# jianzhnie/RLZero

Measured on AMD Instinct MI355X. Metric: mcts_sims_per_sec, higher is better.
Workload: dtype f32 net (hi + lo f16 operand pairs on the f16 MFMA pipe, f32 accumulation) / f64 tree

## Files before the change

profiles/microbench/delta_resident_phases.py:

```python
import ctypes, os, sys
sys.path.insert(0, os.environ.get('GRAFT_REPO_ROOT', '.'))
import rlzero_amd._hip as H
H.library_path = lambda: os.environ.get('RZ_NETPROF_LIB') or os.path.join(os.path.dirname(os.path.abspath(__file__)), 'librlzero_netprof.so')
import rlzero_amd._build as B
B.needs_build = lambda: False
import numpy as np, torch
from rlzero_amd.engine import HipNetEvaluator, MCTSEngine
from rlzero_amd.games.gomoku.policy_value_net import PolicyValueNet
lib = H.load()
NAMES = [(0, 'leaf + changed cells'), (1, 'distances, requests, ranks'), (3, 'maps, base records'), (4, 'bar'), (5, 'conv1'), (6, 'bar'), (7, 'conv2'),
         (9, 'bar + conv3 + heads'), (10, 'bar'), (11, 'features'), (12, 'bar'), (16, 'value layer'), (17, 'expand + backup'),
         (2, 'sel: root record'), (8, 'sel: root scan / answer'), (13, 'sel: level-0 cell'), (14, 'sel: deeper levels'), (15, 'sel: terminal test + leaf stores'),
         (18, 'selection (rest: hand-over)'), (19, 'wave 1: pre-scan'), (20, 'wave 1: wait behind it')]
VALUES = '--values' in sys.argv[1:]
if VALUES:
    import rlzero_amd.route as _R
    _R.policy_on_demand = lambda *a, **k: True
sizes = [int(a) for a in sys.argv[1:] if a != '--values'] or [1, 256, 512]
for games in sizes:
    torch.manual_seed(0)
    net = PolicyValueNet(15).to('cuda:0')
    ev = HipNetEvaluator(net, 15, 'cuda:0', max_boards=games)
    sims = 800
    eng = MCTSEngine(15, 5, n_games=games, n_playout=sims, device='cuda:0', add_noise=True)
    eng.reset_games()
    assert ev.resident_ok(eng) and ev.resident_delta_ok(eng)
    rng = np.random.default_rng(0)
    for ply in range(6):
        eng.sim_chunk(ev, 40)
        visits = eng.root_visits()
        moves = np.array([int(rng.choice(np.flatnonzero(v > 0))) for v in visits], dtype=np.int32)
        eng.advance(moves)
        eng.step(moves)
    a, b = torch.cuda.Event(enable_timing=True), torch.cuda.Event(enable_timing=True)
    ev.hip.delta_stats(reset=True)
    a.record(); eng.sim_chunk(ev, sims); b.record(); torch.cuda.synchronize()
    assert (eng.search_launches[True] > 0) == VALUES and (eng.search_launches[False] > 0) != VALUES
    st = ev.hip.delta_stats()
    out = (ctypes.c_longlong * 24)()
    assert lib.rz_net_debug_profile(out) == 0
    us = 1e3 * a.elapsed_time(b) / sims
    total = out[23] / sims
    print('%d games, %d simulations: %.2f us per simulation of a game (events, bases included), %d cycles (%.2f GHz); %.2f conv3 / %.2f conv2 tiles, %.2f changed cells per leaf, %d leaves without a base' % (
        games, sims, us, total, total / us / 1e3, st['tiles3'] / max(1, st['delta'] + st['no_base']), st['tiles2'] / max(1, st['delta'] + st['no_base']),
        st['cells'] / max(1, st['delta'] + st['no_base']), st['no_base']))
    print('   ' + '  '.join('%s=%d' % (nm, out[k] / sims) for k, nm in NAMES) + '  prescans=%d' % st['prescans'], flush=True)
    eng.close(); ev.hip.close()
```

rlzero_amd/csrc/rz_delta.h:

```cpp

#pragma once

#include <hip/hip_runtime.h>

#include <stdint.h>

#include "rlzero_hip.h"
#include "rz_gather.h"
#include "rz_net_dev.h"
#include "rz_net_rows.h"
#include "rz_net_split.h"
#include "rz_trace.h"
#include "rz_tree.h"
#include "rz_window.h"

#ifndef RZ_DELTA_TREE_PRIO
#define RZ_DELTA_TREE_PRIO 1
#endif
#ifndef RZ_DELTA_PRO_PRIO
#define RZ_DELTA_PRO_PRIO 0
#endif
#ifndef RZ_DELTA_PRESCAN
#define RZ_DELTA_PRESCAN 1
#endif

namespace {

namespace dl {

using sp::f16x4;
using sp::f16x8;
typedef const __attribute__((address_space(3))) f16x8 *lds_frag;
typedef const __attribute__((address_space(3))) uint32_t *lds_u32;
typedef __attribute__((address_space(3))) f16x4 *lds_h4;
typedef __attribute__((address_space(3))) f32x4 *lds_v4;

constexpr int kC1Slots = 128, kC2Slots = 164;
constexpr int kT1 = 4, kT2 = 8, kT3 = 8;
constexpr int kMaxD = 4;
constexpr int P1 = rt::Geo<32>::pos_bytes, P2 = rt::Geo<64>::pos_bytes;
constexpr int kGrid = kRowW * kRowW;
constexpr int kShareFloats = kT3 * 4 * 96;
constexpr int kHeadW = 128 * 6 * 4 + 128 * 4 + 32;
constexpr int kOffC1 = sp::kInPieceBytes, kOffC2 = kOffC1 + kC1Slots * P1, kOffZero = kOffC2 + kC2Slots * P2, kOffHead = kOffZero + P2,
              kOffMap1 = kOffHead + kHeadW, kOffMap2 = kOffMap1 + kGrid * 4, kOffList = kOffMap2 + kGrid * 4,
              kLdsBytes = kOffList + 3 * 128 * 2;
static_assert(kShareFloats * 4 <= kC1Slots * P1, "the shares lie inside conv1's records (dead behind conv2)");
constexpr int kWinSets = rzw::kRadii * rzw::kWords, kWinLds = kWinSets * 8 + kWinSets * 4 + 16;
static_assert(2 * (kLdsBytes + 512 * 4 + 4 * 64 * 4 + 80 + kWinLds + (int)sizeof(rzt::RootPre) + 512) <= 160 * 1024,
              "two workgroups per CU, also of the resident search (value row, K-quarter sums, leaf, window sets, root pre-scan)");
static_assert(kOffC1 % 16 == 0 && kOffZero % 16 == 0 && kOffHead % 16 == 0 && kOffMap1 % 16 == 0, "alignment");

constexpr int kCells = RZ_MAX_BOARD_SIZE * RZ_MAX_BOARD_SIZE;
struct BaseHdr {
    uint64_t stones[2 * RZ_BOARD_WORDS];
    int32_t to_move, valid, pad[2];
};
constexpr size_t kBaseC2 = (size_t)kCells * 128, kBaseV = kBaseC2 + (size_t)kCells * 256, kBaseBytes = kBaseV + (size_t)6 * kCells * 4;

struct DeltaArgs {
    BaseHdr *hdr;
    char *recs;
    const uint8_t *active;
    float *feat32;
    unsigned *stats;
    int mode;
    int bw_rcp;
    const uint64_t *win;
};

__device__ __forceinline__ uint32_t lds_addr(const void *p) {
    return (uint32_t)(uintptr_t)((const __attribute__((address_space(3))) char *)p);
}

constexpr int unit_tiles(int nt) { return nt <= 3 ? nt : (nt + 1) / 2; }
constexpr int units_of(int nt) { return (nt + unit_tiles(nt) - 1) / unit_tiles(nt); }

template <int CIN, int NT, int UT>
__device__ __forceinline__ void read_unit(f16x8 (&b)[UT][2], const uint32_t (&rec)[NT][3], int h, int dy, int c) {
#pragma unroll
    for (int i = 0; i < UT; ++i) {
        const int t = h * UT + i;
        if (t < NT) {
            const uint32_t r = rec[t][dy] + (uint32_t)(c * 64);
            b[i][0] = *(lds_frag)(uintptr_t)r;
            b[i][1] = *(lds_frag)(uintptr_t)(r + CIN * 2);
        }
    }
}
template <int TM, int NT, int UT>
__device__ __forceinline__ void mfma_unit(f32x4 (&acc)[TM][NT], const f16x8 (&a)[TM][2], const f16x8 (&b)[UT][2], int h) {
#pragma unroll
    for (int combo = 0; combo < 3; ++combo)
#pragma unroll
        for (int i = 0; i < UT; ++i) {
            const int t = h * UT + i;
            if (t < NT) {
#pragma unroll
                for (int m = 0; m < TM; ++m)
                    acc[m][t] = __builtin_amdgcn_mfma_f32_16x16x32_f16(a[m][combo == 2], b[i][combo == 1], acc[m][t], 0, 0, 0);
            }
        }
}
template <int NT>
__device__ __forceinline__ void lookup(uint32_t (&rec)[NT][3], lds_u32 map, const int (&pos19)[NT], int dx, int g) {
#pragma unroll
    for (int t = 0; t < NT; ++t)
#pragma unroll
        for (int dy = 0; dy < 3; ++dy) rec[t][dy] = map[pos19[t] + dx + dy * kRowW] + (uint32_t)(g * 16);
}

template <int NT>
__device__ __forceinline__ void conv2_g(lds_u32 map, const int (&pos19)[NT], int lane, const f16x8 (&a2)[9][1][2], f32x4 (&acc)[1][NT]) {
    static_assert(NT <= 4, "one unit per step");
    const int g = lane >> 4;
#pragma unroll
    for (int t = 0; t < NT; ++t) acc[0][t] = f32x4{0.f, 0.f, 0.f, 0.f};
    constexpr int AHEAD = NT <= 2 ? 2 : 1;
    uint32_t rec[3][NT][3];
    f16x8 b[AHEAD + 1][NT][2];
#pragma unroll
    for (int dx = 0; dx < 3; ++dx) lookup<NT>(rec[dx], map, pos19, dx, g);
#pragma unroll
    for (int u = 0; u < AHEAD; ++u) read_unit<32, NT, NT>(b[u], rec[u / 3], 0, u % 3, 0);
#pragma unroll
    for (int u = 0; u < 9; ++u) {
        const int dx = u / 3, dy = u % 3;
        if (u + AHEAD < 9) read_unit<32, NT, NT>(b[(u + AHEAD) % (AHEAD + 1)], rec[(u + AHEAD) / 3], 0, (u + AHEAD) % 3, 0);
        mfma_unit<1, NT, NT>(acc, a2[dy * 3 + dx], b[u % (AHEAD + 1)], 0);
        __builtin_amdgcn_sched_barrier(0);
    }
}

#ifndef RZ_DELTA_RING6_UPTO
#define RZ_DELTA_RING6_UPTO 2
#endif
constexpr int ring3(int nt) { return nt <= RZ_DELTA_RING6_UPTO ? 6 : 3; }
__device__ __forceinline__ void load_a3(f16x8 (&a)[2][2], __amdgpu_buffer_rsrc_t w_rsrc, int lane, int dx, int j) {
    using G = rt::Geo<64>;
    const int c = j / 3, dy = j % 3;
#pragma unroll
    for (int m = 0; m < 2; ++m)
#pragma unroll
        for (int p = 0; p < 2; ++p)
            a[m][p] = sp::load_w(w_rsrc, lane * 16, dx * (G::chunks * 2048) + ((m * G::steps + dy * 3 * G::chunks + c) * 2 + p) * 1024);
}
template <int NT>
__device__ __forceinline__ void conv3_g(lds_u32 map, const uint16_t *list3, const void *wts, int lane, bool sync, f32x4 (&acc)[2][NT]) {
    static_assert(NT <= 6, "two units per step");
    constexpr int R = ring3(NT), H = units_of(NT);
    const int n = lane & 15, g = lane >> 4;
    const __amdgpu_buffer_rsrc_t w_rsrc = __builtin_amdgcn_make_buffer_rsrc(const_cast<void *>(wts), 0, 0x7fffffff, 0x00020000);
    f16x8 a3[R][2][2];
#pragma unroll
    for (int j = 0; j < R - 1; ++j) load_a3(a3[j], w_rsrc, lane, 0, j);
    if (sync) __syncthreads();
    int pos19[NT];
#pragma unroll
    for (int t = 0; t < NT; ++t) pos19[t] = (int)list3[16 * t + n] - 19;
#pragma unroll
    for (int m = 0; m < 2; ++m)
#pragma unroll
        for (int t = 0; t < NT; ++t) acc[m][t] = f32x4{0.f, 0.f, 0.f, 0.f};
    uint32_t rec[NT][3], recn[NT][3];
#ifndef RZ_DELTA_AHEAD3_SMALL
#define RZ_DELTA_AHEAD3_SMALL 1
#endif
    constexpr int UT = unit_tiles(NT), AH = UT <= 2 ? RZ_DELTA_AHEAD3_SMALL : 1, NB = AH + 1;
    static_assert((6 * H) % NB == 0 && AH <= H * 6, "a unit's registers are a constant of the unrolled body");
    f16x8 b[NB][UT][2];
    lookup<NT>(rec, map, pos19, 0, g);
#pragma unroll
    for (int u = 0; u < AH; ++u) read_unit<64, NT, UT>(b[u], rec, u % H, (u / H) % 3, u / H / 3);
#pragma unroll 1
    for (int dx = 0; dx < 3; ++dx) {
        lookup<NT>(recn, map, pos19, dx < 2 ? dx + 1 : 2, g);
#pragma unroll
        for (int u = 0; u < 6 * H; ++u) {
            const int j = u / H, h = u % H;
            if (h == 0) {
                const int jj = j + R - 1, dx2 = jj < 6 ? dx : (dx < 2 ? dx + 1 : 2);
                load_a3(a3[jj % R], w_rsrc, lane, dx2, jj % 6);
            }
            {
                const int v = u + AH;
                if (v < 6 * H) read_unit<64, NT, UT>(b[v % NB], rec, v % H, (v / H) % 3, v / H / 3);
                else read_unit<64, NT, UT>(b[v % NB], recn, (v - 6 * H) % H, ((v - 6 * H) / H) % 3, (v - 6 * H) / H / 3);
            }
            mfma_unit<2, NT, UT>(acc, a3[j % R], b[u % NB], h);
            __builtin_amdgcn_sched_barrier(0);
        }
#pragma unroll
        for (int t = 0; t < NT; ++t)
#pragma unroll
            for (int dy = 0; dy < 3; ++dy) rec[t][dy] = recn[t][dy];
    }
}

template <int T, int O = 6>
__device__ __forceinline__ void reduce_scatter(const float (&vals)[O * T], float (&out)[O * T / 4]) {
    float r1[O * T / 2];
#pragma unroll
    for (int i = 0; i < O * T / 2; ++i) {
        const auto sw = __builtin_amdgcn_permlane16_swap(__float_as_uint(vals[i]), __float_as_uint(vals[O * T / 2 + i]), false, false);
        r1[i] = __uint_as_float(sw[0]) + __uint_as_float(sw[1]);
    }
#pragma unroll
    for (int i = 0; i < O * T / 4; ++i) {
        const auto sw = __builtin_amdgcn_permlane32_swap(__float_as_uint(r1[i]), __float_as_uint(r1[O * T / 4 + i]), false, false);
        out[i] = __uint_as_float(sw[0]) + __uint_as_float(sw[1]);
    }
}

template <int NT>
__device__ __forceinline__ void conv2_tiles(lds_u32 map1, lds_u32 map2, const uint16_t *list2, int n2, int lane, int wave, const f16x8 (&a2)[9][1][2],
                                            f32x4 bias2, float k2) {
    const int n = lane & 15, g = lane >> 4;
    int pos19[NT];
#pragma unroll
    for (int t = 0; t < NT; ++t) pos19[t] = (int)list2[16 * t + n] - 19;
    f32x4 acc[1][NT];
    conv2_g<NT>(map1, pos19, lane, a2, acc);
#pragma unroll
    for (int t = 0; t < NT; ++t) {
        if (16 * t + n < n2) {
            const uint32_t rec = map2[pos19[t] + kRowW + 1] + (uint32_t)((16 * wave + 4 * g) * 2);
            float z[4];
#pragma unroll
            for (int j = 0; j < 4; ++j) z[j] = fmaxf(fmaf(acc[0][t][j], k2, bias2[j]), 0.0f);
            f16x4 hi, lo;
            sp::split4(z, hi, lo);
            *(lds_h4)(uintptr_t)rec = hi;
            *(lds_h4)(uintptr_t)(rec + 128) = lo;
        }
    }
}

template <int NT, int OLO = 0, int OHI = 6>
__device__ __forceinline__ void conv3_tiles(lds_u32 map2, const uint16_t *list3, const void *wts, int lane, int wave, bool sync,
                                            const char *headw, float k3, float *shares) {
    constexpr int T = NT <= 4 ? 4 : 8, O = OHI - OLO;
    static_assert(OLO % 2 == 0 && OHI % 2 == 0 && 0 <= OLO && OLO < OHI && OHI <= 6, "pairs of outputs");
    const int n = lane & 15, g = lane >> 4;
    float vals[O * T];
    {
        f32x4 acc[2][NT];
        conv3_g<NT>(map2, list3, wts, lane, sync, acc);
        f32x4 hwr[2][6], b3r[2];
#pragma unroll
        for (int m = 0; m < 2; ++m) {
            const int c0 = 32 * wave + 16 * m + 4 * g;
#pragma unroll
            for (int i = 0; i < 6; ++i) hwr[m][i] = *reinterpret_cast<const f32x4 *>(headw + (c0 * 6 + 4 * i) * 4);
            b3r[m] = *reinterpret_cast<const f32x4 *>(headw + 128 * 6 * 4 + c0 * 4);
        }
#pragma unroll
        for (int t = 0; t < T; ++t) {
            f32x2 v2[3] = {f32x2{0.0f, 0.0f}, f32x2{0.0f, 0.0f}, f32x2{0.0f, 0.0f}};
            if (t < NT) {
#pragma unroll
                for (int m = 0; m < 2; ++m)
#pragma unroll
                    for (int j = 0; j < 4; ++j) {
                        const float hv = fmaxf(fmaf(acc[m][t < NT ? t : 0][j], k3, b3r[m][j]), 0.0f);
#pragma unroll
                        for (int o2 = OLO / 2; o2 < OHI / 2; ++o2) {
                            const int e = 6 * j + 2 * o2;
                            v2[o2] = __builtin_elementwise_fma(f32x2{hwr[m][e >> 2][e & 3], hwr[m][e >> 2][(e & 3) + 1]}, f32x2{hv, hv}, v2[o2]);
                        }
                    }
            }
#pragma unroll
            for (int o = OLO; o < OHI; ++o) vals[t * O + o - OLO] = v2[o >> 1][o & 1];
        }
    }
    float mine[O * T / 4];
    reduce_scatter<T, O>(vals, mine);
    const int t0 = (T / 2) * (g & 1) + (T / 4) * (g >> 1);
#pragma unroll
    for (int i = 0; i < O * T / 4; ++i)
        if (t0 + i / O < NT) shares[((t0 + i / O) * 4 + wave) * 96 + (OLO + i % O) * 16 + n] = mine[i];
}

struct Leaf {
    f16x4 cell_planes;
    const char *base;
    int dys[kMaxD], dxs[kMaxD];
    _Float16 *dst16;
    float *vdst;
    float *dst32;
    const uint64_t *sets;
    uint16_t *gtab;
    bool deferred, store_head;
};
struct Layers {
    float k1, k2, k3, act1, act2, act3;
    const char *t2p, *t3p;
};
#ifdef RZ_NET_PROFILE
struct Prof { long long acc[24], t; };
#else
struct Prof {};
#endif

__device__ __forceinline__ void init_maps(char *lds, int tid) {
    uint32_t *map1 = reinterpret_cast<uint32_t *>(lds + kOffMap1);
    const uint32_t zaddr = lds_addr(lds + kOffZero);
    for (int i = tid; i < 2 * kGrid; i += 256) map1[i] = zaddr;
    if (tid < 3 * 128 / 2) reinterpret_cast<uint32_t *>(lds + kOffList)[tid] = 19u | (19u << 16);
}

__device__ __forceinline__ int cell_dist(int cy, int cx, int pass, const int (&dys)[kMaxD], const int (&dxs)[kMaxD], int BH, int BW) {
    int dist = 1000;
    if (pass < 0) {
#pragma unroll
        for (int i = 0; i < kMaxD; ++i) {
            const int ady = cy > dys[i] ? cy - dys[i] : dys[i] - cy, adx = cx > dxs[i] ? cx - dxs[i] : dxs[i] - cx;
            const int d = ady > adx ? ady : adx;
            dist = d < dist ? d : dist;
        }
    } else {
        const int y0 = 8 * (pass >> 1), x0 = 8 * (pass & 1);
        const int y1 = (y0 + 8 < BH ? y0 + 8 : BH) - 1, x1 = (x0 + 8 < BW ? x0 + 8 : BW) - 1;
        const int ddy = cy < y0 ? y0 - cy : (cy > y1 ? cy - y1 : 0), ddx = cx < x0 ? x0 - cx : (cx > x1 ? cx - x1 : 0);
        dist = ddy > ddx ? ddy : ddx;
    }
    return dist;
}

constexpr int kOutside = 1 << 30;
__device__ __forceinline__ f32x4 load_rec(__amdgpu_buffer_rsrc_t rsrc, int off) {
    return __builtin_bit_cast(f32x4, __builtin_amdgcn_raw_buffer_load_b128(rsrc, off, 0, 0));
}

__device__ __forceinline__ uint64_t uni64(uint64_t v) {
    return ((uint64_t)(unsigned)__builtin_amdgcn_readfirstlane((int)(v >> 32)) << 32) | (unsigned)__builtin_amdgcn_readfirstlane((int)v);
}

__device__ __forceinline__ int lane_below(uint64_t word) {
    return (int)__builtin_amdgcn_mbcnt_hi((unsigned)(word >> 32), __builtin_amdgcn_mbcnt_lo((unsigned)word, 0u));
}
static_assert(rzg::kC1Max == kC1Slots && rzg::kC2Max == kC2Slots && rzg::kC1Bytes * kCells == (int)kBaseC2 && rzg::kOutside == kOutside,
              "rz_gather.h's records are the base's and the budget is this file's");
static_assert(rzg::kC1Bytes <= P1 && rzg::kC2Bytes <= P2, "a record fits its LDS slot");

template <bool SETS, int OLO = 0, int OHI = 6>
__device__ __forceinline__ int delta_passes(const NetDev &nd, const DeltaArgs &da, char *lds, int tid0, int wave, const Leaf &leaf, const Layers &ly,
                                            f32x4 headv, bool &use_delta, Prof &prof) {
    char *in0 = lds, *c1 = lds + kOffC1, *c2 = lds + kOffC2, *zrec = lds + kOffZero, *headw = lds + kOffHead;
    uint32_t *map1 = reinterpret_cast<uint32_t *>(lds + kOffMap1), *map2 = reinterpret_cast<uint32_t *>(lds + kOffMap2);
    uint16_t *list1 = reinterpret_cast<uint16_t *>(lds + kOffList), *list2 = list1 + 128, *list3 = list2 + 128;
    float *shares = reinterpret_cast<float *>(c1);
    const int mode = da.mode, BH = nd.BH, BW = nd.BW, S = nd.S;
    const float k1 = ly.k1, k2 = ly.k2, k3 = ly.k3, act1 = ly.act1, act2 = ly.act2, act3 = ly.act3;
    const char *t2p = ly.t2p, *t3p = ly.t3p;
    const char *base = leaf.base;
    const f16x4 cell_planes = leaf.cell_planes;
    const int (&dys)[kMaxD] = leaf.dys, (&dxs)[kMaxD] = leaf.dxs;
    _Float16 *dst16 = leaf.dst16;
    float *vdst = leaf.vdst, *dst32 = leaf.dst32;
    const bool deferred = leaf.deferred, store_head = leaf.store_head;
    const uint32_t zaddr = lds_addr(zrec);
    int n_conv3_tiles = 0, n_conv2_tiles = 0;
#ifdef RZ_NET_PROFILE
    long long (&prof_acc)[24] = prof.acc, &prof_t = prof.t;
#endif
    for (int pass = use_delta ? -1 : 0; pass < 4; ++pass) {
        int tid = tid0;
        asm volatile("" : "+v"(tid));
        const int lane = tid & 63, g = lane >> 4;
        const int cy = (tid * da.bw_rcp) >> 16, cx = tid - cy * BW;
        const bool is_cell = tid < S;
        const int mypos = is_cell ? (cy + 1) * kRowW + cx + 1 : 0;
        if (RZ_DELTA_PRO_PRIO) __builtin_amdgcn_s_setprio(RZ_DELTA_PRO_PRIO);
        const int th[5] = {pass < 0 ? 1 : 2, pass < 0 ? 2 : 1, pass < 0 ? 3 : 0, pass < 0 ? 3 : 2, pass < 0 ? 4 : 1};
        bool f[5];
        uint64_t own[5];
        const bool handed = SETS && pass < 0;
        int rank[5], tot[5];
        if (handed) {
#pragma unroll
            for (int k = 0; k < 5; ++k) {
                own[k] = uni64(leaf.sets[4 * (th[k] - 1) + wave]);
                f[k] = (own[k] >> lane) & 1ull;
            }
            const int *cnt = reinterpret_cast<const int *>(leaf.sets + kWinSets);
#pragma unroll
            for (int k = 0; k < 5; ++k) {
                int before = 0, all = 0;
#pragma unroll
                for (int w = 0; w < 4; ++w) {
                    const int c = __builtin_amdgcn_readfirstlane(cnt[4 * (th[k] - 1) + w]);
                    all += c;
                    before += w < wave ? c : 0;
                }
                rank[k] = before + (int)__builtin_amdgcn_mbcnt_hi((unsigned)(own[k] >> 32), __builtin_amdgcn_mbcnt_lo((unsigned)own[k], 0u));
                tot[k] = all;
            }
        } else {
            const int dist = cell_dist(cy, cx, pass, dys, dxs, BH, BW);
#pragma unroll
            for (int k = 0; k < 5; ++k) f[k] = is_cell && dist <= th[k];
        }
        const bool g1 = pass < 0 && f[3] && !f[0], g2 = pass < 0 && f[4] && !f[1];
        const __amdgpu_buffer_rsrc_t b_rsrc = __builtin_amdgcn_make_buffer_rsrc(const_cast<char *>(base), 0, kBaseBytes, 0x00020000);
        f32x4 r1[8], r2[16];
        f32x4 q1[rzg::kC1Rounds], q2[rzg::kC2Rounds];
        uint32_t d1[rzg::kC1Rounds], d2[rzg::kC2Rounds];
        if constexpr (SETS) {
            uint16_t *tab = leaf.gtab;
            uint64_t ws[rzw::kRadii][rzg::kWords];
#pragma unroll
            for (int r = 0; r < rzw::kRadii; ++r)
#pragma unroll
                for (int w = 0; w < rzg::kWords; ++w) ws[r][w] = leaf.sets[4 * r + w];
            int n1 = 0, s1 = 0, n2 = 0, s2 = 0;
#pragma unroll
            for (int w = 0; w < rzg::kWords; ++w) {
                const uint64_t h1 = rzg::held(ws[2][w], ws[0][w]), h2 = rzg::held(ws[3][w], ws[1][w]);
                const int cell = 64 * w + lane;
                const int p1 = rzg::c1_place(n1 + lane_below(h1), wave), p2 = rzg::c2_place(n2 + lane_below(h2), wave);
                const uint16_t e1 = rzg::entry(cell, s1 + lane_below(ws[2][w])), e2 = rzg::entry(cell, s2 + lane_below(ws[3][w]));
                if (handed && ((h1 >> lane) & 1ull) && p1 >= 0) tab[p1] = e1;
                if (handed && ((h2 >> lane) & 1ull) && p2 >= 0) tab[p2] = e2;
                n1 += rzg::popcount(h1), s1 += rzg::popcount(ws[2][w]);
                n2 += rzg::popcount(h2), s2 += rzg::popcount(ws[3][w]);
            }
            const uint32_t c1a = lds_addr(c1), c2a = lds_addr(c2);
#pragma unroll
            for (int i = 0; i < rzg::kC1Rounds; ++i) {
                const int j = rzg::c1_record(i, wave, lane), chunk = rzg::c1_chunk(lane);
                const uint16_t e = tab[rzg::c1_index(j)];
                const bool has = handed && rzg::c1_has(j, n1);
                d1[i] = has ? c1a + (uint32_t)rzg::dst(rzg::entry_slot(e), chunk, P1) : zaddr + 16u * (uint32_t)chunk;
                q1[i] = load_rec(b_rsrc, rzg::c1_src(has, rzg::entry_cell(e), chunk));
            }
#pragma unroll
            for (int i = 0; i < rzg::kC2Rounds; ++i) {
                const int j = rzg::c2_record(i, wave, lane), chunk = rzg::c2_chunk(lane);
                const uint16_t e = tab[rzg::c2_index(j)];
                const bool has = handed && rzg::c2_has(j, n2);
                d2[i] = has ? c2a + (uint32_t)rzg::dst(rzg::entry_slot(e), chunk, P2) : zaddr + 16u * (uint32_t)chunk;
                q2[i] = load_rec(b_rsrc, rzg::c2_src(has, rzg::entry_cell(e), chunk, (int)kBaseC2));
            }
        } else {
            const int o1 = g1 ? tid * 128 : kOutside, o2 = g2 ? (int)kBaseC2 + tid * 256 : kOutside;
#pragma unroll
            for (int i = 0; i < 8; ++i) r1[i] = load_rec(b_rsrc, o1 + 16 * i);
#pragma unroll
            for (int i = 0; i < 16; ++i) r2[i] = load_rec(b_rsrc, o2 + 16 * i);
        }
        float bv[6];
        {
            const int ov = pass < 0 && is_cell && !f[2] ? (int)kBaseV + tid * 4 : kOutside;
#pragma unroll
            for (int o = OLO; o < OHI; ++o) bv[o] = __builtin_bit_cast(float, __builtin_amdgcn_raw_buffer_load_b32(b_rsrc, ov + o * kCells * 4, 0, 0));
        }
        sp::f16x8 a1[3][2];
        f32x4 bias1[4];
        if constexpr (SETS) {
            const __amdgpu_buffer_rsrc_t s_rsrc = __builtin_amdgcn_make_buffer_rsrc(const_cast<f32x4 *>(nd.s1), 0, 6 * 64 * 16, 0x00020000);
            const __amdgpu_buffer_rsrc_t o_rsrc = __builtin_amdgcn_make_buffer_rsrc(const_cast<float *>(nd.b1), 0, 32 * 4, 0x00020000);
            const bool runs = !handed || 32 * wave < tot[0];
            const int so = runs ? lane * 16 : kOutside, bo = runs ? 16 * (lane >> 5) : kOutside;
#pragma unroll
            for (int ky = 0; ky < 3; ++ky)
#pragma unroll
                for (int p_ = 0; p_ < 2; ++p_) a1[ky][p_] = sp::load_w(s_rsrc, so, (ky * 2 + p_) * 1024);
#pragma unroll
            for (int gg = 0; gg < 4; ++gg) bias1[gg] = load_rec(o_rsrc, bo + 32 * gg);
        } else if (32 * wave < 32 * kT1) {
#pragma unroll
            for (int ky = 0; ky < 3; ++ky)
#pragma unroll
                for (int p_ = 0; p_ < 2; ++p_) a1[ky][p_] = __builtin_bit_cast(sp::f16x8, nd.s1[(ky * 2 + p_) * 64 + lane]);
#pragma unroll
            for (int gg = 0; gg < 4; ++gg) bias1[gg] = *reinterpret_cast<const f32x4 *>(nd.b1 + 8 * gg + 4 * (lane >> 5));
        }
        f32x4 bias2 = *reinterpret_cast<const f32x4 *>(nd.b2 + 16 * wave + 4 * g);
        if (!handed) {
            int before[5] = {0, 0, 0, 0, 0}, all[5] = {0, 0, 0, 0, 0};
            unsigned long long own[5] = {0ull, 0ull, 0ull, 0ull, 0ull};
#pragma unroll
            for (int b = 0; b < 4; ++b) {
                const int cell = 64 * b + lane, by = (cell * da.bw_rcp) >> 16, bx = cell - by * BW;
                const int d = cell_dist(by, bx, pass, dys, dxs, BH, BW);
#pragma unroll
                for (int k = 0; k < 5; ++k) {
                    const unsigned long long m = __ballot(cell < S && d <= th[k]);
                    const int c = __popcll(m);
                    all[k] += c;
                    before[k] += b < wave ? c : 0;
                    own[k] = b == wave ? m : own[k];
                }
            }
#pragma unroll
            for (int k = 0; k < 5; ++k) {
                rank[k] = before[k] + (int)__builtin_amdgcn_mbcnt_hi((unsigned)(own[k] >> 32), __builtin_amdgcn_mbcnt_lo((unsigned)own[k], 0u));
                tot[k] = all[k];
            }
        }
        NET_TICK(1);
        if (pass < 0 && (tot[0] > 32 * kT1 || tot[1] > 16 * kT2 || tot[2] > 16 * kT3 || tot[3] > kC1Slots || tot[4] > kC2Slots)) {
            use_delta = false;
            continue;
        }
        uint32_t rec1 = 0, rec2 = 0;
        if (f[3]) {
            rec1 = lds_addr(c1 + rank[3] * P1);
            map1[mypos] = rec1;
        }
        if (f[4]) {
            rec2 = lds_addr(c2 + rank[4] * P2);
            map2[mypos] = rec2;
        }
        if (f[0]) list1[rank[0]] = (uint16_t)mypos;
        if (f[1]) list2[rank[1]] = (uint16_t)mypos;
        if (f[2]) list3[rank[2]] = (uint16_t)mypos;
        if (pass <= 0 && is_cell) *reinterpret_cast<f16x4 *>(in0 + ((cy + 1) * sp::kInCols + (cx + 1)) * 8) = cell_planes;
        if (pass <= 0 && store_head && tid < 226) reinterpret_cast<f32x4 *>(headw)[tid] = headv;
        if constexpr (SETS) {
#pragma unroll
            for (int i = 0; i < rzg::kC1Rounds; ++i) *(lds_v4)(uintptr_t)d1[i] = q1[i];
#pragma unroll
            for (int i = 0; i < rzg::kC2Rounds; ++i) *(lds_v4)(uintptr_t)d2[i] = q2[i];
        } else {
            if (g1) {
#pragma unroll
                for (int i = 0; i < 8; ++i) *(lds_v4)(uintptr_t)(rec1 + 16 * i) = r1[i];
            }
            if (g2) {
#pragma unroll
                for (int i = 0; i < 16; ++i) *(lds_v4)(uintptr_t)(rec2 + 16 * i) = r2[i];
            }
        }
        __builtin_amdgcn_sched_barrier(0);
        f16x8 a2[9][1][2];
        {
            const __amdgpu_buffer_rsrc_t w_rsrc = __builtin_amdgcn_make_buffer_rsrc(const_cast<char *>(t2p), 0, 0x7fffffff, 0x00020000);
#pragma unroll
            for (int tap = 0; tap < 9; ++tap)
#pragma unroll
                for (int p = 0; p < 2; ++p) a2[tap][0][p] = sp::load_w(w_rsrc, lane * 16, (tap * 2 + p) * 1024);
        }
        NET_TICK(3);
        __syncthreads();
        NET_TICK(4);

        if (32 * wave < tot[0]) {
            const int n32 = lane & 31, h = lane >> 5, idx = 32 * wave + n32;
            const int pos = list1[idx];
            const int py = (pos * 3641) >> 16, px = pos - py * kRowW;
            typedef const __attribute__((address_space(3))) f16x4 *lds_half;
            const lds_half q = (lds_half)(in0 + ((py - 1) * sp::kInCols + (px - 1) + 2 * h) * 8);
            sp::f16x8 b1[3];
#pragma unroll
            for (int ky = 0; ky < 3; ++ky) {
                const int o = ky * sp::kInCols;
                const f16x4 lo4 = q[o], hi4 = q[o + 1];
                b1[ky] = __builtin_shufflevector(lo4, hi4, 0, 1, 2, 3, 4, 5, 6, 7);
            }
            sp::f32x16 acc1;
#pragma unroll
            for (int r = 0; r < 16; ++r) acc1[r] = 0.0f;
#pragma unroll
            for (int ky = 0; ky < 3; ++ky)
#pragma unroll
                for (int combo = 0; combo < 3; combo += 2)
                    acc1 = __builtin_amdgcn_mfma_f32_32x32x16_f16(a1[ky][combo == 2], b1[ky], acc1, 0, 0, 0);
            if (idx < tot[0]) {
                const uint32_t rec = map1[pos] + (uint32_t)(4 * h * 2);
#pragma unroll
                for (int gg = 0; gg < 4; ++gg) {
                    float z[4];
#pragma unroll
                    for (int j = 0; j < 4; ++j) z[j] = fmaxf(fmaf(acc1[4 * gg + j], k1, bias1[gg][j] * act1), 0.0f);
                    f16x4 hi, lo;
                    sp::split4(z, hi, lo);
                    *(lds_h4)(uintptr_t)(rec + 8 * gg * 2) = hi;
                    *(lds_h4)(uintptr_t)(rec + 8 * gg * 2 + 64) = lo;
                }
            }
        }
        NET_TICK(5);
        __syncthreads();
        NET_TICK(6);
        if (mode == 1 && f[0]) {
            f32x4 *dstp = reinterpret_cast<f32x4 *>(const_cast<char *>(base) + (size_t)tid * 128);
#pragma unroll
            for (int i = 0; i < 8; ++i) dstp[i] = *(lds_v4)(uintptr_t)(rec1 + 16 * i);
        }

        if (RZ_DELTA_PRO_PRIO) __builtin_amdgcn_s_setprio(0);
        const int nt3 = (tot[2] + 15) >> 4;
        {
            const lds_u32 m1 = (lds_u32)map1, m2 = (lds_u32)map2;
            const int nt2 = (tot[1] + 15) >> 4;
            n_conv2_tiles += nt2;
            for (int t0 = 0; t0 < nt2; t0 += 4) {
                const uint16_t *l2 = list2 + 16 * t0;
                const int left = tot[1] - 16 * t0;
                switch (nt2 - t0) {
                    case 1: conv2_tiles<1>(m1, m2, l2, left, lane, wave, a2, bias2 * act2, k2); break;
                    case 2: conv2_tiles<2>(m1, m2, l2, left, lane, wave, a2, bias2 * act2, k2); break;
                    case 3: conv2_tiles<3>(m1, m2, l2, left, lane, wave, a2, bias2 * act2, k2); break;
                    default: conv2_tiles<4>(m1, m2, l2, left, lane, wave, a2, bias2 * act2, k2); break;
                }
            }
        }
        NET_TICK(7);

        {
            const lds_u32 m2 = (lds_u32)map2;
            n_conv3_tiles += nt3;
            const int first = nt3 <= 6 ? nt3 : 4;
            switch (first) {
                case 0: __syncthreads(); break;
                case 1: conv3_tiles<1, OLO, OHI>(m2, list3, t3p, lane, wave, true, headw, k3, shares); break;
                case 2: conv3_tiles<2, OLO, OHI>(m2, list3, t3p, lane, wave, true, headw, k3, shares); break;
                case 3: conv3_tiles<3, OLO, OHI>(m2, list3, t3p, lane, wave, true, headw, k3, shares); break;
                case 4: conv3_tiles<4, OLO, OHI>(m2, list3, t3p, lane, wave, true, headw, k3, shares); break;
                case 5: conv3_tiles<5, OLO, OHI>(m2, list3, t3p, lane, wave, true, headw, k3, shares); break;
                default: conv3_tiles<6, OLO, OHI>(m2, list3, t3p, lane, wave, true, headw, k3, shares); break;
            }
            if (nt3 == 7) conv3_tiles<3, OLO, OHI>(m2, list3 + 64, t3p, lane, wave, false, headw, k3, shares + 4 * 4 * 96);
            else if (nt3 >= 8) conv3_tiles<4, OLO, OHI>(m2, list3 + 64, t3p, lane, wave, false, headw, k3, shares + 4 * 4 * 96);
        }
        NET_TICK(9);
        __syncthreads();
        NET_TICK(10);
        if (mode == 1 && f[1]) {
            f32x4 *dstp = reinterpret_cast<f32x4 *>(const_cast<char *>(base) + kBaseC2 + (size_t)tid * 256);
#pragma unroll
            for (int i = 0; i < 16; ++i) dstp[i] = *(lds_v4)(uintptr_t)(rec2 + 16 * i);
        }

        if (is_cell && (pass < 0 || f[2])) {
            const float *share = shares + (rank[2] >> 4) * 4 * 96 + (rank[2] & 15);
            float *basev = mode == 1 ? reinterpret_cast<float *>(const_cast<char *>(base) + kBaseV) : nullptr;
#pragma unroll
            for (int o = OLO; o < OHI; ++o) {
                float v;
                if (f[2]) {
                    float s = share[o * 16];
#pragma unroll
                    for (int w = 1; w < 4; ++w) s += share[w * 96 + o * 16];
                    v = fmaxf(s + reinterpret_cast<const float *>(headw + 128 * 7 * 4)[o], 0.0f);
                } else {
                    v = bv[o];
                }
                if (mode == 1) {
                    basev[o * kCells + tid] = v;
                    continue;
                }
                if (dst32) dst32[o * S + tid] = v;
                if (deferred && o >= 4) {
                    vdst[(o - 4) * S + tid] = v;
                } else if (dst16) {
                    const int k = (o < 4 ? o : o - 4) * S + tid;
                    const int step = (o < 4 ? 0 : nd.groups_act) + (k >> 4);
                    const float z = v * act3;
                    const _Float16 zh = (_Float16)z;
                    _Float16 *q = dst16 + (size_t)step * 1024 + (k & 15);
                    q[0] = zh;
                    q[512] = (_Float16)(z - (float)zh);
                }
            }
        }
        if (f[3]) map1[mypos] = zaddr;
        if (f[4]) map2[mypos] = zaddr;
        NET_TICK(11);
        if (pass < 0) break;
        __syncthreads();
    }
    return n_conv3_tiles | (n_conv2_tiles << 16);
}

__device__ __forceinline__ f16x4 planes_of(const uint64_t (&ls)[8], int tid, int tm_eff, bool has_last, int lc, int par_count) {
    f16x4 cell_planes;
    const int word = (tid >> 6) & 3, bit = tid & 63;
    uint64_t w0 = 0ull, w1 = 0ull;
#pragma unroll
    for (int w = 0; w < 4; ++w) {
        const uint64_t mk = word == w ? ~0ull : 0ull;
        w0 |= ls[w] & mk;
        w1 |= ls[4 + w] & mk;
    }
    const bool s0 = (w0 >> bit) & 1ull, s1 = (w1 >> bit) & 1ull;
    const bool mine = tm_eff == 0 ? s0 : s1, theirs = tm_eff == 0 ? s1 : s0;
    const _Float16 one = (_Float16)sp::kObsScale, zero = (_Float16)0.0f;
    cell_planes[0] = mine ? one : zero;
    cell_planes[1] = theirs ? one : zero;
    cell_planes[2] = (has_last && tid == lc) ? one : zero;
    cell_planes[3] = (par_count & 1) ? zero : one;
    return cell_planes;
}

__device__ __forceinline__ bool changed_cells(const uint64_t (&ls)[8], const uint64_t (&rs)[8], int nst, int tm, int lc, bool has_last, bool base_ok, int h_tm,
                                              int bw_rcp, int BW, int (&dys)[kMaxD], int (&dxs)[kMaxD], int &parity, int &nD) {
    bool use_delta = false;
    {
        bool sup = true;
        int nroot = 0;
        uint64_t D[4] = {0ull, 0ull, 0ull, 0ull};
#pragma unroll
        for (int q = 0; q < 8; ++q) {
            sup = sup && (rs[q] & ~ls[q]) == 0ull;
            nroot += __popcll(rs[q]);
            D[q & 3] |= rs[q] ^ ls[q];
        }
#pragma unroll
        for (int w = 0; w < 4; ++w) D[w] |= (has_last && lc >= 0 && (lc >> 6) == w) ? 1ull << (lc & 63) : 0ull;
        parity = (nst - nroot) & 1;
        nD = __popcll(D[0]) + __popcll(D[1]) + __popcll(D[2]) + __popcll(D[3]);
        use_delta = base_ok && sup && tm == (h_tm ^ parity) && nD <= kMaxD;
#pragma unroll
        for (int i = 0; i < kMaxD; ++i) {
            const bool z0 = D[0] == 0ull, z1 = D[1] == 0ull, z2 = D[2] == 0ull;
            const int w = !z0 ? 0 : !z1 ? 1 : !z2 ? 2 : 3;
            const uint64_t word = !z0 ? D[0] : !z1 ? D[1] : !z2 ? D[2] : D[3];
            const bool any = word != 0ull;
            const int cell = 64 * w + __builtin_ctzll(word | (1ull << 63));
            const uint64_t rest = word & (word - 1ull);
#pragma unroll
            for (int k = 0; k < 4; ++k) D[k] = k == w ? rest : D[k];
            const int y = (cell * bw_rcp) >> 16;
            dys[i] = any ? y : -100;
            dxs[i] = any ? cell - y * BW : -100;
        }
    }
    return use_delta;
}

template <bool TRACE>
__global__ __launch_bounds__(256, 2) void k_trunk_delta(NetDev nd, LeafBits leaves, _Float16 *__restrict__ feat16, int n_boards,
                                                        DeferredOut later, DeltaArgs da) {
    __shared__ __attribute__((aligned(16))) char lds[kLdsBytes];
    const int board = blockIdx.x;
    const int mode = da.mode;
    const int game = mode == 1 ? board >> 1 : board, par_b = mode == 1 ? board & 1 : 0;
    unsigned long long trace_t0 = 0;
    if (TRACE) trace_t0 = rz_trace_now();
    Prof prof;
#ifdef RZ_NET_PROFILE
    for (int i = 0; i < 24; ++i) prof.acc[i] = 0;
    prof.t = __builtin_readcyclecounter();
    const long long prof_k0 = prof.t;
    long long (&prof_acc)[24] = prof.acc, &prof_t = prof.t;
#endif
    const int tid0 = threadIdx.x, wave = __builtin_amdgcn_readfirstlane(tid0 >> 6);
    const int BW = nd.BW, S = nd.S;
    Layers ly;
    ly.t2p = reinterpret_cast<const char *>(nd.t2) + (size_t)wave * rt::Geo<32>::steps * 2 * 1024;
    ly.t3p = reinterpret_cast<const char *>(nd.t3) + (size_t)(2 * wave) * rt::Geo<64>::steps * 2 * 1024;
    f32x4 headv = tid0 < 192 ? reinterpret_cast<const f32x4 *>(nd.whp)[tid0] : reinterpret_cast<const f32x4 *>(nd.b3)[(tid0 - 192) & 31];
    {
        const float *bh = nd.bh + (tid0 == 225 ? 4 : 0);
        const f32x4 hbv = {bh[0], bh[1], tid0 == 225 ? 0.0f : bh[2], tid0 == 225 ? 0.0f : bh[3]};
        headv = (tid0 == 224 || tid0 == 225) ? hbv : headv;
    }
    ly.k1 = nd.s_inv[2], ly.k2 = nd.s_inv[0], ly.k3 = nd.s_inv[1];
    ly.act1 = nd.s_inv[5], ly.act2 = nd.s_inv[6], ly.act3 = nd.s_inv[7];

    const uint64_t *sb = leaves.stones + (size_t)game * 8;
    const BaseHdr *hd = da.hdr + game;
    uint64_t ls[8], rs[8];
    int nst = 0;
#pragma unroll
    for (int q = 0; q < 8; ++q) {
        ls[q] = sb[q];
        rs[q] = hd->stones[q];
        nst += __popcll(ls[q]);
    }
    const int tm = leaves.to_move[game];
    const int lc_raw = (mode == 1 ? leaves.to_move : leaves.last)[game];
    const int lc = mode == 1 ? -1 : lc_raw;
    const int h_tm = hd->to_move, h_valid = hd->valid;
    const int is_active = da.active[game];
    const bool deferred = later.slot_of != nullptr;
    const int slot_ = (deferred ? later.slot_of : leaves.to_move)[deferred ? board : game];
    const int tm_eff = tm ^ par_b;
    const int par_count = nst + par_b;
    const bool has_last = mode != 1 && nst > 0;

    Leaf leaf;
    int parity = 0, nD = 0;
    bool use_delta = changed_cells(ls, rs, nst, tm, lc, has_last, mode == 0 && h_valid != 0, h_tm, da.bw_rcp, BW, leaf.dys, leaf.dxs, parity, nD);
    leaf.base = da.recs + ((size_t)game * 2 + (mode == 1 ? par_b : parity)) * kBaseBytes;
    leaf.cell_planes = planes_of(ls, tid0, tm_eff, has_last, lc, par_count);

    leaf.dst16 = nullptr;
    leaf.vdst = nullptr;
    if (mode != 1 && deferred) {
        leaf.dst16 = (feat16 != nullptr && slot_ < later.n_slots) ? feat16 + (size_t)slot_ * later.slot_halfs + (size_t)(board >> 5) * nd.groups_act * 1024 + (board & 31) * 16 : nullptr;
        leaf.vdst = later.valfeat + (size_t)board * later.vf_ld;
    }
    if (mode != 1 && !deferred && feat16 != nullptr)
        leaf.dst16 = feat16 + ((size_t)(board >> 5) * (nd.groups_act + nd.groups_val) * 1024 + (board & 31) * 16);
    leaf.dst32 = (mode != 1 && da.feat32 != nullptr) ? da.feat32 + (size_t)board * 6 * S : nullptr;
    leaf.sets = nullptr, leaf.gtab = nullptr;
    leaf.deferred = deferred;
    leaf.store_head = true;

    {
        const f32x4 zero = {0.f, 0.f, 0.f, 0.f};
        f32x4 *z = reinterpret_cast<f32x4 *>(lds);
        for (int i = tid0; i < sp::kInPieceBytes / 16; i += 256) z[i] = zero;
        if (tid0 < P2 / 16) reinterpret_cast<f32x4 *>(lds + kOffZero)[tid0] = zero;
        init_maps(lds, tid0);
    }
    if (mode == 0 && is_active == 0) return;
    __syncthreads();
    NET_TICK(0);
    const int n_tiles = delta_passes<false>(nd, da, lds, tid0, wave, leaf, ly, headv, use_delta, prof);
    const int n_conv3_tiles = n_tiles & 0xffff;

    if (mode == 1 && par_b == 0 && tid0 == 0) {
        BaseHdr *h = da.hdr + game;
#pragma unroll
        for (int q = 0; q < 8; ++q) h->stones[q] = sb[q];
        h->to_move = tm;
        h->valid = 1;
    }
    if (da.stats != nullptr && tid0 == 0 && mode != 1) {
        atomicAdd(da.stats + (use_delta ? 0 : 1), 1u);
        atomicAdd(da.stats + 2, (unsigned)n_conv3_tiles);
        atomicAdd(da.stats + 3, (unsigned)nD);
        atomicAdd(da.stats + 4, (unsigned)(n_tiles >> 16));
    }
#ifdef RZ_NET_PROFILE
    if (blockIdx.x == 0 && tid0 == 0) {
        for (int i = 0; i < 24; ++i) net_prof[i] = prof_acc[i];
        net_prof[23] = __builtin_readcyclecounter() - prof_k0;
        net_prof[22] = n_conv3_tiles;
    }
#endif
    if (TRACE && tid0 == 0) rz_trace_write(later.trace, RZ_TRACE_TRUNK, deferred ? slot_ : 0, board, trace_t0);
}

__device__ __forceinline__ void windows_store(uint64_t row, bool use_delta, int parity, int nD, int lane, uint64_t *ws) {
    unsigned lo = (unsigned)row, hi = (unsigned)(row >> 32);
    {
        const auto a = __builtin_amdgcn_permlane16_swap(lo, lo, false, false), b = __builtin_amdgcn_permlane16_swap(hi, hi, false, false);
        lo = a[0] | a[1];
        hi = b[0] | b[1];
    }
    {
        const auto a = __builtin_amdgcn_permlane32_swap(lo, lo, false, false), b = __builtin_amdgcn_permlane32_swap(hi, hi, false, false);
        lo = a[0] | a[1];
        hi = b[0] | b[1];
    }
    const uint64_t v = ((uint64_t)hi << 32) | lo;
    int *cnt = reinterpret_cast<int *>(ws + kWinSets);
    if (lane < kWinSets) {
        ws[lane] = v;
        cnt[lane] = __popcll(v);
    }
    if (lane == 0) cnt[kWinSets] = (use_delta ? 1 : 0) | (parity << 1) | (nD << 8);
}
__device__ __forceinline__ void leaf_windows(const uint64_t *leaf_lds, const uint64_t (&rs)[8], bool base_ok, int h_tm, const DeltaArgs &da, int BW,
                                             int lane, uint64_t *ws) {
    uint64_t ls[8];
    int nst = 0;
#pragma unroll
    for (int q = 0; q < 8; ++q) {
        ls[q] = uni64(leaf_lds[q]);
        nst += __popcll(ls[q]);
    }
    const int tm = __builtin_amdgcn_readfirstlane(reinterpret_cast<const int *>(leaf_lds + 2 * RZ_BOARD_WORDS)[0]);
    const int lc = __builtin_amdgcn_readfirstlane(reinterpret_cast<const int *>(leaf_lds + 2 * RZ_BOARD_WORDS)[1]);
    int dys[kMaxD], dxs[kMaxD], parity = 0, nD = 0;
    const bool use_delta = changed_cells(ls, rs, nst, tm, lc, nst > 0, base_ok, h_tm, da.bw_rcp, BW, dys, dxs, parity, nD);
    const int i = lane >> 4;
    int dy = dys[0], dx = dxs[0];
#pragma unroll
    for (int j = 1; j < kMaxD; ++j) {
        dy = i == j ? dys[j] : dy;
        dx = i == j ? dxs[j] : dx;
    }
    const bool any = dy >= 0;
    const uint64_t row = da.win[(any ? dy * BW + dx : 0) * kWinSets + (lane & (kWinSets - 1))];
    windows_store(any ? row : 0ull, use_delta, parity, nD, lane, ws);
}

#if defined(RZ_NET_PROFILE) && !defined(RZ_SEL_TICKS)
#define RZ_SEL_TICKS 0
#endif
struct ResHook {
    static constexpr bool kOn = true;
    rzt::RootPre *pre;
    const uint64_t *win;
    int depth;
    bool any0;
    uint64_t row;
    __device__ __forceinline__ void root_cell(int last, int stones, int lane) {
        any0 = stones > 0 && last >= 0 && last < kCells;
        row = win[(any0 ? last : 0) * kWinSets + (lane & (kWinSets - 1))];
    }
    __device__ __forceinline__ void cell(int level, int c, int lane) {
        const uint64_t v = win[c * kWinSets + (lane & (kWinSets - 1))];
        row = (lane >> 4) == level ? v : row;
    }
#ifdef RZ_NET_PROFILE
    Prof *prof;
    __device__ __forceinline__ void tick(int i, int arrived) {
        if ((RZ_SEL_TICKS >> i) & 1) {
            asm volatile("" ::"v"(arrived));
            const int slot = i == 0 ? 2 : i == 1 ? 8 : 12 + i;
            __builtin_amdgcn_sched_barrier(0);
            const long long now = __builtin_readcyclecounter();
            prof->acc[slot] += now - prof->t;
            prof->t = now;
            __builtin_amdgcn_sched_barrier(0);
        }
    }
#else
    __device__ __forceinline__ void tick(int, int) {}
#endif
};

__device__ __forceinline__ void path_windows(const ResHook &hook, bool base_ok, int lane, uint64_t *ws) {
    const int depth = hook.depth;
    const bool mine = depth == 0 ? (lane < 16 && hook.any0) : (lane >> 4) < depth;
    const int nD = depth == 0 ? (hook.any0 ? 1 : 0) : depth;
    windows_store(mine ? hook.row : 0ull, base_ok && nD <= kMaxD, depth & 1, nD, lane, ws);
}

constexpr int kResVrow = 512;
template <bool POL>
__global__ __launch_bounds__(256, 2) void k_delta_res(NetDev nd, _Float16 *__restrict__ store16, DeferredOut later, DeltaArgs da, ResArgs<true> res) {
    __shared__ __attribute__((aligned(16))) char lds[kLdsBytes];
    __shared__ float res_vrow[kResVrow];
    __shared__ float res_part[rzt::kDefWaves][rzt::kWave];
    static_assert(rzg::kTabEntries * 2 <= rzt::kWave * 4, "a wave's gather table lies in its row of the K-quarter sums");
    __shared__ __attribute__((aligned(16))) uint64_t res_leaf[2 * RZ_BOARD_WORDS + 2];
    __shared__ __attribute__((aligned(16))) uint64_t res_win[kWinLds / 8];
    __shared__ __attribute__((aligned(16))) rzt::RootPre res_pre;
    const int game = res.order != nullptr ? res.order[blockIdx.x] : (int)blockIdx.x;
    if ((unsigned)game >= (unsigned)res.E.n_games || res.E.active[game] == 0) return;
    const int n_sims = res_sims(res, game);
    const unsigned long long clk0 = __builtin_readcyclecounter(), rt0 = __builtin_amdgcn_s_memrealtime();
    const int tid0 = threadIdx.x, wave = __builtin_amdgcn_readfirstlane(tid0 >> 6);
    const int BW = nd.BW;
    Prof prof;
#ifdef RZ_NET_PROFILE
    for (int i = 0; i < 24; ++i) prof.acc[i] = 0;
    prof.t = __builtin_readcyclecounter();
    const long long prof_k0 = prof.t;
    long long (&prof_acc)[24] = prof.acc, &prof_t = prof.t;
#endif
    Layers ly;
    ly.t2p = reinterpret_cast<const char *>(nd.t2) + (size_t)wave * rt::Geo<32>::steps * 2 * 1024;
    ly.t3p = reinterpret_cast<const char *>(nd.t3) + (size_t)(2 * wave) * rt::Geo<64>::steps * 2 * 1024;
    f32x4 headv = tid0 < 192 ? reinterpret_cast<const f32x4 *>(nd.whp)[tid0] : reinterpret_cast<const f32x4 *>(nd.b3)[(tid0 - 192) & 31];
    {
        const float *bh = nd.bh + (tid0 == 225 ? 4 : 0);
        const f32x4 hbv = {bh[0], bh[1], tid0 == 225 ? 0.0f : bh[2], tid0 == 225 ? 0.0f : bh[3]};
        headv = (tid0 == 224 || tid0 == 225) ? hbv : headv;
    }
    ly.k1 = nd.s_inv[2], ly.k2 = nd.s_inv[0], ly.k3 = nd.s_inv[1];
    ly.act1 = nd.s_inv[5], ly.act2 = nd.s_inv[6], ly.act3 = nd.s_inv[7];
    const int slot0 = res.E.pend[game];
    uint64_t rs[8];
    bool base_ok = da.hdr[game].valid != 0;
#pragma unroll
    for (int q = 0; q < 8; ++q) {
        rs[q] = res.E.root_stones[(size_t)game * 8 + q];
        base_ok = base_ok && da.hdr[game].stones[q] == rs[q];
    }
    const int h_tm = res.E.root_to_move[game];
    base_ok = base_ok && da.hdr[game].to_move == h_tm;
    {
        const f32x4 zero = {0.f, 0.f, 0.f, 0.f};
        f32x4 *z = reinterpret_cast<f32x4 *>(lds);
        for (int i = tid0; i < sp::kInPieceBytes / 16; i += 256) z[i] = zero;
        if (tid0 < P2 / 16) reinterpret_cast<f32x4 *>(lds + kOffZero)[tid0] = zero;
        init_maps(lds, tid0);
        for (int i = tid0; i < kResVrow; i += 256) res_vrow[i] = 0.0f;
    }
    if (tid0 == 0) res_pre.scan = res_pre.valid = res_pre.answered = 0;
    ResHook hook;
    hook.pre = &res_pre;
    hook.win = da.win;
    hook.depth = 0;
    hook.any0 = false;
    hook.row = 0ull;
#ifdef RZ_NET_PROFILE
    hook.prof = &prof;
    long long pre_cycles = 0, pre_wait = 0;
#endif
    if (res.select_first == 0 && tid0 == 0) {
#pragma unroll
        for (int q = 0; q < 8; ++q) res_leaf[q] = res.E.leaf_stones[(size_t)game * 8 + q];
        reinterpret_cast<int *>(res_leaf + 2 * RZ_BOARD_WORDS)[0] = res.E.leaf_to_move[game];
        reinterpret_cast<int *>(res_leaf + 2 * RZ_BOARD_WORDS)[1] = res.E.leaf_last[game];
    }
    __syncthreads();
    if (wave == 0) {
        const int lane0 = tid0 & 63;
        if (res.select_first != 0) {
            rzt::select_body<false, rzt::kWords, ResHook>(res.E, nullptr, game, lane0, 0, res_leaf, &hook);
            path_windows(hook, base_ok, lane0, res_win);
        } else {
            leaf_windows(res_leaf, rs, base_ok, h_tm, da, BW, lane0, res_win);
        }
    }
    __syncthreads();
    int tiles_total = 0, tiles2_total = 0, deltas = 0, cells_total = 0;
    for (int sim = 0; sim < n_sims; ++sim) {
        int tid_s = tid0;
        asm volatile("" : "+v"(tid_s));
        uint64_t ls[8];
        int nst = 0;
#pragma unroll
        for (int q = 0; q < 8; ++q) {
            const uint64_t v = res_leaf[q];
            ls[q] = ((uint64_t)(unsigned)__builtin_amdgcn_readfirstlane((int)(v >> 32)) << 32) | (unsigned)__builtin_amdgcn_readfirstlane((int)v);
            nst += __popcll(ls[q]);
        }
        const int tm = __builtin_amdgcn_readfirstlane(reinterpret_cast<const int *>(res_leaf + 2 * RZ_BOARD_WORDS)[0]);
        const int lc = __builtin_amdgcn_readfirstlane(reinterpret_cast<const int *>(res_leaf + 2 * RZ_BOARD_WORDS)[1]);
        const bool has_last = nst > 0;
        const int verdict = __builtin_amdgcn_readfirstlane(reinterpret_cast<const int *>(res_win + kWinSets)[kWinSets]);
        bool use_delta = (verdict & 1) != 0;
        const int parity = (verdict >> 1) & 1, nD = verdict >> 8;
        Leaf leaf;
        leaf.sets = res_win;
        leaf.gtab = reinterpret_cast<uint16_t *>(res_part[wave]);
#pragma unroll
        for (int i = 0; i < kMaxD; ++i) leaf.dys[i] = leaf.dxs[i] = -100;
        leaf.base = da.recs + ((size_t)game * 2 + parity) * kBaseBytes;
        leaf.cell_planes = planes_of(ls, tid_s, tm, has_last, lc, nst);
        leaf.dst16 = POL && slot0 + sim < later.n_slots ? store16 + (size_t)(slot0 + sim) * later.slot_halfs + (size_t)(game >> 5) * nd.groups_act * 1024 + (game & 31) * 16 : nullptr;
        leaf.vdst = res_vrow;
        leaf.dst32 = nullptr;
        leaf.deferred = true;
        leaf.store_head = sim == 0;
        NET_TICK(0);
        const int n_tiles = delta_passes<true, POL ? 0 : 4, 6>(nd, da, lds, tid_s, wave, leaf, ly, headv, use_delta, prof);
        tiles_total += n_tiles & 0xffff;
        tiles2_total += n_tiles >> 16;
        deltas += use_delta ? 1 : 0;
        cells_total += nD;
        __syncthreads();
        NET_TICK(12);
        const int lane = tid_s & 63;
        if (RZ_DELTA_TREE_PRIO) __builtin_amdgcn_s_setprio(RZ_DELTA_TREE_PRIO);
        if (res.vh.groups == 128) rzt::value_quarter_lds<16>(res.vh, res_vrow, lane, wave, res_part);
        else rzt::value_quarter_lds<8>(res.vh, res_vrow, lane, wave, res_part);
        NET_TICK(16);
        const bool more = sim + 1 < n_sims;
        if (wave == 0) {
            rzt::expand_backup_body<float, false, false, false, true>(res.E, nullptr, nullptr, game, lane, rz_raw_heads(), 0, res.vh, res_part);
        } else {
            __syncthreads();
            if (RZ_DELTA_PRESCAN && wave == 1 && more) {
#ifdef RZ_NET_PROFILE
                const long long t0 = __builtin_readcyclecounter();
#endif
                rzt::root_prescan<rzt::kWords>(res.E, game, lane, &res_pre);
#ifdef RZ_NET_PROFILE
                __builtin_amdgcn_s_waitcnt(0);
                const long long t1 = __builtin_readcyclecounter();
                pre_cycles += t1 - t0;
                pre_wait -= t1;
#endif
            }
        }
        __syncthreads();
#ifdef RZ_NET_PROFILE
        if (RZ_DELTA_PRESCAN && wave == 1 && more) pre_wait += __builtin_readcyclecounter();
#endif
        NET_TICK(17);
        if (wave == 0 && more) {
            hook.depth = 0, hook.any0 = false, hook.row = 0ull;
            int lane_t = lane;
            asm volatile("" : "+v"(lane_t));
            rzt::select_body<false, rzt::kWords, ResHook>(res.E, nullptr, game, lane_t, 0, res_leaf, &hook);
            path_windows(hook, base_ok, lane_t, res_win);
        }
        if (RZ_DELTA_TREE_PRIO) __builtin_amdgcn_s_setprio(0);
        __syncthreads();
        NET_TICK(18);
    }
    if (da.stats != nullptr && tid0 == 0) {
        atomicAdd(da.stats + 0, (unsigned)deltas);
        atomicAdd(da.stats + 1, (unsigned)(n_sims - deltas));
        atomicAdd(da.stats + 2, (unsigned)tiles_total);
        atomicAdd(da.stats + 3, (unsigned)cells_total);
        atomicAdd(da.stats + 4, (unsigned)tiles2_total);
        atomicAdd(da.stats + 5, (unsigned)res_pre.answered);
        if (game == 0) {
            da.stats[6] = (unsigned)((__builtin_readcyclecounter() - clk0) >> 8);
            da.stats[7] = (unsigned)(__builtin_amdgcn_s_memrealtime() - rt0);
        }
    }
#ifdef RZ_NET_PROFILE
    if (blockIdx.x == 0 && tid0 == 0) {
        for (int i = 0; i < 24; ++i)
            if (i != 19 && i != 20) net_prof[i] = prof_acc[i];
        net_prof[23] = __builtin_readcyclecounter() - prof_k0;
        net_prof[22] = tiles_total;
    }
    if (blockIdx.x == 0 && tid0 == 64) {
        net_prof[19] = pre_cycles;
        net_prof[20] = pre_wait;
    }
#endif
}

struct PolicyRows {
    const int32_t *rows, *count;
    const uint64_t *stones;
    const int32_t *lw;
    int n_games, n_slots;
    long long slot_halfs;
};
__global__ __launch_bounds__(256, 2) void k_trunk_policy_rows(NetDev nd, _Float16 *__restrict__ store16, DeltaArgs da, PolicyRows pr) {
    __shared__ __attribute__((aligned(16))) char lds[kLdsBytes];
    const int tid0 = threadIdx.x, wave = __builtin_amdgcn_readfirstlane(tid0 >> 6);
    const int BW = nd.BW;
    Prof prof;
#ifdef RZ_NET_PROFILE
    for (int i = 0; i < 24; ++i) prof.acc[i] = 0;
    prof.t = __builtin_readcyclecounter();
#endif
    Layers ly;
    ly.t2p = reinterpret_cast<const char *>(nd.t2) + (size_t)wave * rt::Geo<32>::steps * 2 * 1024;
    ly.t3p = reinterpret_cast<const char *>(nd.t3) + (size_t)(2 * wave) * rt::Geo<64>::steps * 2 * 1024;
    f32x4 headv = tid0 < 192 ? reinterpret_cast<const f32x4 *>(nd.whp)[tid0] : reinterpret_cast<const f32x4 *>(nd.b3)[(tid0 - 192) & 31];
    {
        const float *bh = nd.bh + (tid0 == 225 ? 4 : 0);
        const f32x4 hbv = {bh[0], bh[1], tid0 == 225 ? 0.0f : bh[2], tid0 == 225 ? 0.0f : bh[3]};
        headv = (tid0 == 224 || tid0 == 225) ? hbv : headv;
    }
    ly.k1 = nd.s_inv[2], ly.k2 = nd.s_inv[0], ly.k3 = nd.s_inv[1];
    ly.act1 = nd.s_inv[5], ly.act2 = nd.s_inv[6], ly.act3 = nd.s_inv[7];
    const int n_rows = pr.count[0];
    {
        const f32x4 zero = {0.f, 0.f, 0.f, 0.f};
        f32x4 *z = reinterpret_cast<f32x4 *>(lds);
        for (int i = tid0; i < sp::kInPieceBytes / 16; i += 256) z[i] = zero;
        if (tid0 < P2 / 16) reinterpret_cast<f32x4 *>(lds + kOffZero)[tid0] = zero;
        init_maps(lds, tid0);
    }
    __syncthreads();
    bool first = true;
    for (int i = blockIdx.x; i < n_rows; i += gridDim.x) {
        int tid_r = tid0;
        asm volatile("" : "+v"(tid_r));
        const int rec = pr.rows[i];
        const int game = rec % pr.n_games, slot = rec / pr.n_games;
        const uint64_t *sb = pr.stones + (size_t)rec * 8;
        const BaseHdr *hd = da.hdr + game;
        uint64_t ls[8], rs[8];
        int nst = 0;
#pragma unroll
        for (int q = 0; q < 8; ++q) {
            ls[q] = sb[q];
            rs[q] = hd->stones[q];
            nst += __popcll(ls[q]);
        }
        const int lw = pr.lw[rec];
        const int h_tm = hd->to_move, h_valid = hd->valid;
        const int tm = rzt::pend_lw_to_move(lw), lc = rzt::pend_lw_last(lw);
        const bool has_last = nst > 0;
        if ((unsigned)slot >= (unsigned)pr.n_slots) continue;
        Leaf leaf;
        int parity = 0, nD = 0;
        bool use_delta = changed_cells(ls, rs, nst, tm, lc, has_last, h_valid != 0, h_tm, da.bw_rcp, BW, leaf.dys, leaf.dxs, parity, nD);
        leaf.base = da.recs + ((size_t)game * 2 + parity) * kBaseBytes;
        leaf.cell_planes = planes_of(ls, tid_r, tm, has_last, lc, nst);
        leaf.dst16 = store16 + (size_t)slot * pr.slot_halfs + (size_t)(game >> 5) * nd.groups_act * 1024 + (game & 31) * 16;
        leaf.vdst = nullptr;
        leaf.dst32 = nullptr;
        leaf.sets = nullptr, leaf.gtab = nullptr;
        leaf.deferred = false;
        leaf.store_head = first;
        first = false;
        (void)delta_passes<false, 0, 4>(nd, da, lds, tid_r, wave, leaf, ly, headv, use_delta, prof);
        __syncthreads();
    }
}

}

}
```

rlzero_amd/csrc/rz_gather.h:

```cpp
#pragma once
#include <stdint.h>

#if defined(__HIPCC__)
#define RZG_FN __host__ __device__ inline
#else
#define RZG_FN inline
#endif

namespace rzg {

constexpr int kWords = 4;
constexpr int kC1Max = 128, kC2Max = 164;
constexpr int kC1Bytes = 128, kC2Bytes = 256;
constexpr int kC1Lanes = kC1Bytes / 16, kC2Lanes = kC2Bytes / 16;
constexpr int kC1PerWave = 64 / kC1Lanes, kC2PerWave = 64 / kC2Lanes;
constexpr int kC1PerRound = 4 * kC1PerWave, kC2PerRound = 4 * kC2PerWave;
constexpr int kC1Rounds = (kC1Max + kC1PerRound - 1) / kC1PerRound;
constexpr int kC2Rounds = (kC2Max + kC2PerRound - 1) / kC2PerRound;
constexpr int kTabC2 = 0, kTabC1 = kC2Rounds * kC2PerWave;
constexpr int kTabEntries = kTabC1 + kC1Rounds * kC1PerWave;
constexpr int kOutside = 1 << 30;

RZG_FN int popcount(uint64_t w) { return __builtin_popcountll(w); }

RZG_FN uint64_t held(uint64_t outer, uint64_t inner) { return outer & ~inner; }
RZG_FN int count(const uint64_t (&m)[kWords]) { return popcount(m[0]) + popcount(m[1]) + popcount(m[2]) + popcount(m[3]); }
RZG_FN int below(uint64_t word, int bit) { return popcount(word & ((1ull << bit) - 1ull)); }
RZG_FN int rank(const uint64_t (&m)[kWords], int cell) {
    int r = 0;
    for (int w = 0; w < kWords; ++w) r += w < (cell >> 6) ? popcount(m[w]) : 0;
    return r + below(m[cell >> 6], cell & 63);
}
RZG_FN int cell_of(const uint64_t (&m)[kWords], int j) {
    for (int w = 0; w < kWords; ++w) {
        uint64_t v = m[w];
        const int c = popcount(v);
        if (j >= c) {
            j -= c;
            continue;
        }
        for (; j > 0; --j) v &= v - 1ull;
        return 64 * w + __builtin_ctzll(v);
    }
    return -1;
}

RZG_FN int c2_record(int round, int wave, int lane) { return kC2PerRound * round + kC2PerWave * wave + (int)((unsigned)lane / kC2Lanes); }
RZG_FN int c2_chunk(int lane) { return (int)((unsigned)lane % kC2Lanes); }
RZG_FN int c1_record(int round, int wave, int lane) { return kC1PerRound * round + kC1PerWave * wave + (int)((unsigned)lane / kC1Lanes); }
RZG_FN int c1_chunk(int lane) { return (int)((unsigned)lane % kC1Lanes); }
RZG_FN int c2_rounds(int n) { return (n + kC2PerRound - 1) / kC2PerRound; }
RZG_FN int c1_rounds(int n) { return (n + kC1PerRound - 1) / kC1PerRound; }

RZG_FN int c2_wave(int j) { return (int)(((unsigned)j / kC2PerWave) % 4u); }
RZG_FN int c2_index(int j) { return kTabC2 + (int)(((unsigned)j / kC2PerRound) * kC2PerWave + (unsigned)j % kC2PerWave); }
RZG_FN int c1_wave(int j) { return (int)(((unsigned)j / kC1PerWave) % 4u); }
RZG_FN int c1_index(int j) { return kTabC1 + (int)(((unsigned)j / kC1PerRound) * kC1PerWave + (unsigned)j % kC1PerWave); }
RZG_FN uint16_t entry(int cell, int slot) { return (uint16_t)(cell | slot << 8); }
RZG_FN int entry_cell(uint16_t e) { return e & 255; }
RZG_FN int entry_slot(uint16_t e) { return e >> 8; }
RZG_FN int c2_place(int j, int wave) { return j < kC2Max && c2_wave(j) == wave ? c2_index(j) : -1; }
RZG_FN int c1_place(int j, int wave) { return j < kC1Max && c1_wave(j) == wave ? c1_index(j) : -1; }

RZG_FN int c2_src(bool has, int cell, int chunk, int base_c2) { return has ? base_c2 + cell * kC2Bytes + 16 * chunk : kOutside; }
RZG_FN int c1_src(bool has, int cell, int chunk) { return has ? cell * kC1Bytes + 16 * chunk : kOutside; }
RZG_FN int dst(int slot, int chunk, int pitch) { return slot * pitch + 16 * chunk; }
RZG_FN bool c2_has(int j, int n) { return j < n && j < kC2Max; }
RZG_FN bool c1_has(int j, int n) { return j < n && j < kC1Max; }

}
```

rlzero_amd/csrc/rz_tree.h:

```cpp
#pragma once
#include <hip/hip_runtime.h>

#include <cmath>
#include <stdint.h>

#include "rlzero_hip.h"
#include "rz_play.h"
#include "rz_trace.h"

#pragma clang fp contract(off)

namespace rzt {
namespace {

constexpr int kWave = 64;
constexpr int kWords = RZ_BOARD_WORDS;

struct Dev {
    int kind, BH, BW, S, A, n_row, n_games, score_mode, n_playout;
    int K;
    int path_stride, qcap;
    long long cap, pcap, logtab_n;
    double c_puct;
    int4 *R;
    float *P;
    int32_t *cur_arena, *top, *ptop, *nblk;
    uint64_t *root_stones;
    int32_t *root_to_move, *root_last;
    uint8_t *active;
    int32_t *path, *leaf_node, *leaf_depth, *leaf_fresh, *leaf_term;
    double *leaf_tval;
    uint64_t *leaf_stones;
    int32_t *leaf_to_move, *leaf_last;
    int32_t *queue;
    int32_t *err, *err_any, *reuse_drops;
    const double *logtab;
    int32_t *noise_ctr;
    uint64_t *noise_key;
    uint64_t noise_seed;
    int add_noise;
    int pend_cap;
    int32_t *pend, *pend_pb, *pend_ctr;
    uint64_t *pend_stones;
    int32_t *pend_lw;
    unsigned long long *trace;
    uint64_t valid[kWords];
    int bw_rcp, n_rcp;
    uint64_t col0;
    const uint64_t *line_tab;
    int line_masks;
};

__host__ __device__ __forceinline__ int pend_lw_pack(int to_move, int last) { return ((last + 1) & 0xffff) | (to_move << 16); }
__host__ __device__ __forceinline__ int pend_lw_to_move(int lw) { return (lw >> 16) & 1; }
__host__ __device__ __forceinline__ int pend_lw_last(int lw) { return (lw & 0xffff) - 1; }

constexpr int kFirstCap = 4;
__device__ __forceinline__ int rec_k(const int4 &lo) { return lo.w & 0xffff; }
__device__ __forceinline__ int rec_cap(const int4 &lo) { return (int)((unsigned)lo.w >> 16); }
__device__ __forceinline__ int pack_kc(int k, int cap) { return k | (cap << 16); }
__device__ __forceinline__ double rec_w(const int4 &hi) { return __hiloint2double(hi.y, hi.x); }
__device__ __forceinline__ int4 make_hi(double w, int pb, float prior) {
    return make_int4(__double2loint(w), __double2hiint(w), pb, __float_as_int(prior));
}
__device__ __forceinline__ int4 *arena_records(const Dev &E, int g, int arena) {
    return E.R + 2 * (((long long)g * 2 + arena) * E.cap);
}
__device__ __forceinline__ float *arena_priors(const Dev &E, int g, int arena) {
    return E.P + ((long long)g * 2 + arena) * E.pcap;
}
__device__ __forceinline__ int32_t *rec_n(int4 *R, int slot) { return reinterpret_cast<int32_t *>(R + 2 * slot); }
__device__ __forceinline__ double *rec_wsum(int4 *R, int slot) { return reinterpret_cast<double *>(R + 2 * slot + 1); }
__device__ __forceinline__ int32_t *rec_pb(int4 *R, int slot) { return reinterpret_cast<int32_t *>(R + 2 * slot + 1) + 2; }

template <int W = kWords>
__device__ __forceinline__ uint64_t word_of(const uint64_t *a, int j) {
    if constexpr (W == 1) return a[0];
    if constexpr (W == 2) {
        const uint64_t m0 = j == 0 ? ~0ull : 0ull;
        return (a[0] & m0) | (a[1] & ~m0);
    }
    const uint64_t m0 = j == 0 ? ~0ull : 0ull, m1 = j == 1 ? ~0ull : 0ull, m2 = j == 2 ? ~0ull : 0ull,
                   m3 = j == 3 ? ~0ull : 0ull;
    return (a[0] & m0) | (a[1] & m1) | (a[2] & m2) | (a[3] & m3);
}
template <int W = kWords>
__device__ __forceinline__ bool test_bit(const uint64_t *a, int c) {
    return (word_of<W>(a, c >> 6) >> (c & 63)) & 1ull;
}
template <int W = kWords>
__device__ __forceinline__ void set_bit(uint64_t *a, int c) {
    const uint64_t m = 1ull << (c & 63);
    if constexpr (W == 1) {
        a[0] |= m;
    } else {
        const int j = c >> 6;
        a[0] |= (j == 0) ? m : 0ull;
        a[1] |= (j == 1) ? m : 0ull;
        if constexpr (W > 2) {
            a[2] |= (j == 2) ? m : 0ull;
            a[3] |= (j == 3) ? m : 0ull;
        }
    }
}
template <int W = kWords>
__device__ __forceinline__ int count_bits(const uint64_t *a) {
    int n = 0;
#pragma unroll
    for (int j = 0; j < W; ++j) n += __popcll(a[j]);
    return n;
}
template <int W = kWords>
__device__ __forceinline__ void load_board(const uint64_t *src, int g, uint64_t (&st)[2][kWords]) {
#pragma unroll
    for (int j = 0; j < kWords; ++j) {
        st[0][j] = j < W ? src[((long long)g * 2 + 0) * kWords + j] : 0ull;
        st[1][j] = j < W ? src[((long long)g * 2 + 1) * kWords + j] : 0ull;
    }
}
template <int W = kWords>
__device__ __forceinline__ void store_board(uint64_t *dst, int g, const uint64_t (&st)[2][kWords], int lane) {
    typedef unsigned long long u64x2 __attribute__((ext_vector_type(2)));
    if (lane < 2) {
        const bool c1 = lane == 1;
        u64x2 lo, hi;
        lo[0] = c1 ? st[1][0] : st[0][0];
        lo[1] = W >= 2 ? (c1 ? st[1][1] : st[0][1]) : 0ull;
        hi[0] = W > 2 ? (c1 ? st[1][2] : st[0][2]) : 0ull;
        hi[1] = W > 2 ? (c1 ? st[1][3] : st[0][3]) : 0ull;
        u64x2 *p = reinterpret_cast<u64x2 *>(dst + ((long long)g * 2 + lane) * kWords);
        p[0] = lo;
        p[1] = hi;
    }
}

struct Legal {
    int k;
    unsigned long long cols;
    int height;
};

template <int W = kWords>
__device__ __forceinline__ Legal legal_of(const Dev &E, const uint64_t *occ, int lane) {
    Legal L;
    L.cols = 0ull;
    L.height = 0;
    if (E.kind == RZ_GAME_CONNECT4) {
        int h = 0;
        if constexpr (W == 1) {
            h = lane < E.BW ? __popcll(occ[0] & (E.col0 << lane)) : 0;
        } else {
            if (lane < E.BW)
                for (int y = 0; y < E.BH; ++y) h += test_bit<W>(occ, y * E.BW + lane) ? 1 : 0;
        }
        L.height = h;
        L.cols = __ballot(lane < E.BW && h < E.BH);
        L.k = __popcll(L.cols);
    } else {
        L.k = E.S - count_bits<W>(occ);
    }
    return L;
}

template <int W = kWords>
__device__ __forceinline__ bool nth_legal(const Dev &E, const uint64_t *occ, const Legal &L, int r, int lane,
                                          int &action, int &cell) {
    if (E.kind == RZ_GAME_CONNECT4) {
        const bool mine = (L.cols >> lane) & 1ull;
        const bool hit = mine && __popcll(L.cols & ((1ull << lane) - 1ull)) == r;
        const unsigned long long m = __ballot(hit);
        if (m == 0ull) return false;
        action = __ffsll((long long)m) - 1;
        cell = __shfl(L.height, action) * E.BW + action;
        return true;
    }
    const uint64_t below = (1ull << lane) - 1ull;
    int before = 0, found = -1;
#pragma unroll
    for (int j = 0; j < W; ++j) {
        const uint64_t e = ~occ[j] & E.valid[j];
        const bool mine = (e >> lane) & 1ull;
        if (mine && before + __popcll(e & below) == r) found = 64 * j + lane;
        before += __popcll(e);
    }
    const unsigned long long m = __ballot(found >= 0);
    if (m == 0ull) return false;
    action = cell = __shfl(found, __ffsll((long long)m) - 1);
    return true;
}

__device__ __forceinline__ bool locate_action(const Dev &E, const uint64_t *occ, const Legal &L, int a,
                                              int &rank, int &cell) {
    if (a < 0 || a >= E.A) return false;
    if (E.kind == RZ_GAME_CONNECT4) {
        if (!((L.cols >> a) & 1ull)) return false;
        rank = __popcll(L.cols & ((1ull << a) - 1ull));
        cell = __shfl(L.height, a) * E.BW + a;
        return true;
    }
    if (test_bit(occ, a)) return false;
    const int i = a >> 6;
    const uint64_t below = (1ull << (a & 63)) - 1ull;
    int r = 0;
#pragma unroll
    for (int j = 0; j < kWords; ++j) {
        const uint64_t e = ~occ[j] & E.valid[j];
        r += (j < i) ? __popcll(e) : ((j == i) ? __popcll(e & below) : 0);
    }
    rank = r;
    cell = a;
    return true;
}

__device__ __forceinline__ int lane_action_rank(const Dev &E, const uint64_t *occ, const Legal &L, int j,
                                                int lane, int &before) {
    if (E.kind == RZ_GAME_CONNECT4) {
        if (j != 0 || !((L.cols >> lane) & 1ull)) return -1;
        return __popcll(L.cols & ((1ull << lane) - 1ull));
    }
    const uint64_t e = ~occ[j] & E.valid[j];
    const int r = ((e >> lane) & 1ull) ? before + __popcll(e & ((1ull << lane) - 1ull)) : -1;
    before += __popcll(e);
    return r;
}

template <int W = kWords>
__device__ __forceinline__ bool line_through(const uint64_t *x, int last, int BH, int BW, int n, int lane, int bw_rcp, int n_rcp,
                                             uint64_t window = 0, uint64_t window_hi = 0, bool masks = false) {
    const int d = (lane * n_rcp) >> 16, t = lane - d * n;
    const int stride = (d == 0) ? 1 : (d == 1) ? BW : (d == 2) ? BW + 1 : BW - 1;
    const int start = last - t * stride, s0 = start < 0 ? 0 : start;
    const int h = (s0 * bw_rcp) >> 16, w = s0 - h * BW;
    const bool right = w <= BW - n, down = h <= BH - n, left = w >= n - 1;
    const bool ok = (d == 0) ? right : (d == 1) ? down : (d == 2) ? (right & down) : (left & down);
    bool all = true;
    if constexpr (W == 1) {
        all = ((x[0] >> s0) & window) == window;
    } else if constexpr (W == 2) {
        const int sh = s0 & 63;
        const uint64_t from0 = (x[0] >> sh) | ((x[1] << 1) << (63 - sh)), from1 = x[1] >> sh;
        const uint64_t v_lo = s0 < 64 ? from0 : from1, v_hi = s0 < 64 ? from1 : 0ull;
        all = ((v_lo & window) == window) & ((v_hi & window_hi) == window_hi);
    } else if (!masks) {
        for (int j = 0; j < n; ++j) all = all & test_bit<W>(x, s0 + j * stride);
    } else {
        const int j0 = s0 >> 6, sh = s0 & 63;
        const uint64_t w_lo = word_of<W>(x, j0), w_hi = word_of<W>(x, j0 + 1);
        const uint64_t v = (w_lo >> sh) | ((w_hi << 1) << (63 - sh));
        all = ((v & window) == window) & test_bit<W>(x, s0 + (n - 1) * stride);
    }
    const bool hit = (lane < 4 * n) & (start >= 0) & ok & all;
    return __ballot(hit) != 0ull;
}

template <int W = kWords>
__device__ __forceinline__ bool line_anywhere(const uint64_t *x, int S, int BH, int BW, int n, int lane, int bw_rcp) {
    bool hit = false;
    for (int m = lane; m < S; m += kWave) {
        if (!test_bit<W>(x, m)) continue;
        const int h = (m * bw_rcp) >> 16, w = m - h * BW;
        const bool right = w <= BW - n, down = h <= BH - n, left = w >= n - 1;
#pragma unroll
        for (int d = 0; d < 4; ++d) {
            const int stride = (d == 0) ? 1 : (d == 1) ? BW : (d == 2) ? BW + 1 : BW - 1;
            const bool ok = (d == 0) ? right : (d == 1) ? down : (d == 2) ? (right && down)
                                                                          : (left && down);
            if (!ok) continue;
            bool all = true;
            for (int j = 1; j < n; ++j) all = all && test_bit<W>(x, m + j * stride);
            hit = hit || all;
        }
    }
    return __ballot(hit) != 0ull;
}

__device__ __forceinline__ void write_obs(float *out, const uint64_t *mine, const uint64_t *theirs,
                                          int last, int nst, int S, int lane) {
    const float colour = (nst & 1) ? 0.0f : 1.0f;
#pragma unroll
    for (int j = 0; j < kWords; ++j) {
        const int c = 64 * j + lane;
        if (c < S) {
            out[c] = (float)((mine[j] >> lane) & 1ull);
            out[S + c] = (float)((theirs[j] >> lane) & 1ull);
            out[2 * S + c] = (nst > 0 && c == last) ? 1.0f : 0.0f;
            out[3 * S + c] = colour;
        }
    }
}

__device__ __forceinline__ void flag(const Dev &E, int g, int bits, int lane) {
    if (lane == 0) {
        atomicOr(&E.err[g], bits);
        atomicOr(E.err_any, bits);
    }
}

__device__ __forceinline__ double uct_ref(double w, int n, double ln_parent, double c) {
    const double nd = (double)n;
    const double q = w / nd;
    const double u = sqrt(ln_parent / nd);
    const double cu = c * u;
    return q + cu;
}

__device__ __forceinline__ double puct(double w, int n, float prior, double sqrt_parent, double c) {
    const double q = n > 0 ? w / (double)n : 0.0;
    const double u = ((double)prior * sqrt_parent) / (double)(n + 1);
    const double cu = c * u;
    return q + cu;
}

using rzplay::mix64;

__device__ __forceinline__ uint32_t hash32(uint32_t x) {
    x ^= x >> 16;
    x *= 0x7feb352du;
    x ^= x >> 15;
    x *= 0x846ca68bu;
    x ^= x >> 16;
    return x;
}

__device__ __forceinline__ float gamma03(uint32_t key) {
    const float d = 1.3f - 1.0f / 3.0f, c = 0.33903103f;
    const float kLn2 = 0.69314718f, k2m24 = 1.0f / 16777216.0f;
    float g = d;
    for (int t = 0; t < 8; ++t) {
        const uint32_t h1 = hash32(key + 3u * t), h2 = hash32(key + 3u * t + 1u), h3 = hash32(key + 3u * t + 2u);
        const float u1 = (float)((h1 >> 8) + 1u) * k2m24;
        const float u2 = (float)(h2 >> 8) * k2m24;
        const float u3 = (float)((h3 >> 8) + 1u) * k2m24;
        const float x = __builtin_amdgcn_sqrtf(-2.0f * kLn2 * __builtin_amdgcn_logf(u1)) * __builtin_amdgcn_cosf(u2);
        float v = 1.0f + c * x;
        if (v <= 0.0f) continue;
        v = v * v * v;
        if (kLn2 * __builtin_amdgcn_logf(u3) < 0.5f * x * x + d - d * v + d * kLn2 * __builtin_amdgcn_logf(v)) {
            g = d * v;
            break;
        }
    }
    const float ub = (float)((hash32(key + 0x5bd1e995u) >> 8) + 1u) * k2m24;
    return g * __builtin_amdgcn_exp2f(__builtin_amdgcn_logf(ub) * (1.0f / 0.3f));
}

template <int CTRL>
__device__ __forceinline__ int dpp_move(int x) { return __builtin_amdgcn_update_dpp(0, x, CTRL, 0xF, 0xF, true); }
template <int STAGE>
__device__ __forceinline__ int partner_of(int x, int lane) {
    if (STAGE == 0) return dpp_move<0xB1>(x);
    if (STAGE == 1) return dpp_move<0x4E>(x);
    if (STAGE == 2) return dpp_move<0x141>(x);
    if (STAGE == 3) return dpp_move<0x140>(x);
    if (STAGE == 4) {
        const auto r = __builtin_amdgcn_permlane16_swap((unsigned)x, (unsigned)x, false, false);
        return (int)((lane & 16) ? r[0] : r[1]);
    }
    const auto r = __builtin_amdgcn_permlane32_swap((unsigned)x, (unsigned)x, false, false);
    return (int)((lane & 32) ? r[0] : r[1]);
}
template <int OFF>
__device__ __forceinline__ float xor_partner(float x, int lane) {
    const int v = __float_as_int(x);
    if (OFF == 32) return __int_as_float(partner_of<5>(v, lane));
    if (OFF == 16) return __int_as_float(partner_of<4>(v, lane));
    if (OFF == 8) return __int_as_float(dpp_move<0x128>(v));
    if (OFF == 4) {
        const int up = dpp_move<0x104>(v), down = dpp_move<0x114>(v);
        return __int_as_float((lane & 4) ? down : up);
    }
    if (OFF == 2) return __int_as_float(dpp_move<0x4E>(v));
    return __int_as_float(dpp_move<0xB1>(v));
}
__device__ __forceinline__ float wave_sum(float x, int lane) {
    x += xor_partner<32>(x, lane);
    x += xor_partner<16>(x, lane);
    x += xor_partner<8>(x, lane);
    x += xor_partner<4>(x, lane);
    x += xor_partner<2>(x, lane);
    x += xor_partner<1>(x, lane);
    return x;
}
__device__ __forceinline__ float wave_max(float x, int lane) {
    x = fmaxf(x, xor_partner<32>(x, lane));
    x = fmaxf(x, xor_partner<16>(x, lane));
    x = fmaxf(x, xor_partner<8>(x, lane));
    x = fmaxf(x, xor_partner<4>(x, lane));
    x = fmaxf(x, xor_partner<2>(x, lane));
    x = fmaxf(x, xor_partner<1>(x, lane));
    return x;
}

template <int STAGE>
__device__ __forceinline__ void max_stage(double &mx, int lane) {
    const long long b = __double_as_longlong(mx);
    const int olo = partner_of<STAGE>((int)b, lane), ohi = partner_of<STAGE>((int)(b >> 32), lane);
    const double ob = __longlong_as_double(((long long)ohi << 32) | (unsigned int)olo);
    mx = ob > mx ? ob : mx;
}
template <int W = kWords>
__device__ __forceinline__ int wave_first_max(double best, int besti, bool wide = true) {
    const int lane = (int)__builtin_amdgcn_mbcnt_hi(~0u, __builtin_amdgcn_mbcnt_lo(~0u, 0u));
    double mx = best;
    max_stage<0>(mx, lane);
    max_stage<1>(mx, lane);
    max_stage<2>(mx, lane);
    max_stage<3>(mx, lane);
    if (wide) {
        max_stage<4>(mx, lane);
        max_stage<5>(mx, lane);
    }
    const bool hit = besti != 0x7fffffff && best == mx;
    constexpr int kSlots = W == 1 ? 1 : (W == 2 ? 2 : 4);
#pragma unroll
    for (int s_ = 0; s_ < kSlots; ++s_) {
        const unsigned long long m = __ballot(hit && (besti >> 6) == s_);
        if (m != 0ull) return 64 * s_ + __ffsll((long long)m) - 1;
    }
    return 0x7fffffff;
}

template <bool SC1>
__device__ __forceinline__ int4 load_half(const int4 *R, int idx) {
    if constexpr (SC1) {
        const __amdgpu_buffer_rsrc_t rsrc = __builtin_amdgcn_make_buffer_rsrc(const_cast<int4 *>(R), 0, 0x7fffffff, 0x00020000);
        const auto v = __builtin_amdgcn_raw_buffer_load_b128(rsrc, idx * 16, 0, 16);
        return make_int4((int)v[0], (int)v[1], (int)v[2], (int)v[3]);
    } else {
        return R[idx];
    }
}
template <bool PUCT, int W = kWords, bool PRE = false>
__device__ __forceinline__ int scan_children(const Dev &E, const int4 *R, const float *P, const int4 &lo,
                                             const int4 &hi, double parent_term, int lane, int4 &clo, int4 &chi,
                                             int skip = -1, double *best_out = nullptr) {
    static_assert(!(PRE && PUCT), "the pre-scan is the reference rule's");
    const int k = rec_k(lo), fc = lo.y, pb = hi.z;
    int4 l0 = make_int4(0, -1, 0, 0), l1 = l0, l2 = l0, l3 = l0;
    int4 h0 = make_int4(0, 0, -1, 0), h1 = h0, h2 = h0, h3 = h0;
    float p0 = 0.f, p1 = 0.f, p2 = 0.f, p3 = 0.f;
    if (lane < k) { l0 = load_half<PRE>(R, 2 * (fc + lane)); h0 = load_half<PRE>(R, 2 * (fc + lane) + 1); if (PUCT) p0 = P[pb + lane]; }
    if constexpr (W >= 2) {
        if (lane + 64 < k) { l1 = load_half<PRE>(R, 2 * (fc + lane + 64)); h1 = load_half<PRE>(R, 2 * (fc + lane + 64) + 1); if (PUCT) p1 = P[pb + lane + 64]; }
    }
    if constexpr (W > 2) {
        if (lane + 128 < k) { l2 = load_half<PRE>(R, 2 * (fc + lane + 128)); h2 = load_half<PRE>(R, 2 * (fc + lane + 128) + 1); if (PUCT) p2 = P[pb + lane + 128]; }
        if (lane + 192 < k) { l3 = load_half<PRE>(R, 2 * (fc + lane + 192)); h3 = load_half<PRE>(R, 2 * (fc + lane + 192) + 1); if (PUCT) p3 = P[pb + lane + 192]; }
    }
    double best = -INFINITY;
    int besti = 0x7fffffff;
    int4 blo = l0, bhi = h0;
    auto consider = [&](const int4 &cl, const int4 &ch, float prior, int r0) {
        bool in = r0 < k;
        if constexpr (PRE) in = in && r0 != skip;
        if (in) {
            const double sc = PUCT ? puct(rec_w(ch), cl.x, prior, parent_term, E.c_puct)
                                   : uct_ref(rec_w(ch), cl.x, parent_term, E.c_puct);
            if (sc > best) {
                best = sc;
                besti = r0;
                blo = cl;
                bhi = ch;
            }
        }
    };
    consider(l0, h0, p0, lane);
    if constexpr (W >= 2) consider(l1, h1, p1, lane + 64);
    if constexpr (W > 2) {
        consider(l2, h2, p2, lane + 128);
        consider(l3, h3, p3, lane + 192);
    }
    const int r = __builtin_amdgcn_readfirstlane(wave_first_max<W>(best, besti, W > 2 || __builtin_amdgcn_readfirstlane(k) > 16));
    if constexpr (PRE) *best_out = -INFINITY;
    if (r >= k) return r;
    const int l = r & 63;
    if constexpr (PRE) {
        const long long b = __double_as_longlong(best);
        *best_out = __hiloint2double(__builtin_amdgcn_readlane((int)(b >> 32), l), __builtin_amdgcn_readlane((int)b, l));
    }
    clo = make_int4(__builtin_amdgcn_readlane(blo.x, l), __builtin_amdgcn_readlane(blo.y, l),
                    __builtin_amdgcn_readlane(blo.z, l), __builtin_amdgcn_readlane(blo.w, l));
    chi = make_int4(__builtin_amdgcn_readlane(bhi.x, l), __builtin_amdgcn_readlane(bhi.y, l),
                    __builtin_amdgcn_readlane(bhi.z, l), __builtin_amdgcn_readlane(bhi.w, l));
    return r;
}

struct RootPre {
    int4 lo;
    int r, scan, arena;
    int answered;
    int4 clo, chi;
    double best, term;
    int besti, valid, pad1[2];
};
struct NoHook { static constexpr bool kOn = false; };

template <int W = kWords>
__device__ __forceinline__ void root_prescan(const Dev &E, int g, int lane, RootPre *pre) {
    const int4 lo = make_int4(__builtin_amdgcn_readfirstlane(pre->lo.x), __builtin_amdgcn_readfirstlane(pre->lo.y),
                              __builtin_amdgcn_readfirstlane(pre->lo.z), __builtin_amdgcn_readfirstlane(pre->lo.w));
    const int r = __builtin_amdgcn_readfirstlane(pre->r), scan = __builtin_amdgcn_readfirstlane(pre->scan);
    const int arena = __builtin_amdgcn_readfirstlane(pre->arena);
    const int n1 = lo.x + 1, k = rec_k(lo);
    const bool ok = scan != 0 && n1 >= 1 && n1 < E.logtab_n && lo.y >= 0 && ((long long)lo.y + k) * 32 < 0x7fffffffll;
    if (ok) {
        const int4 *R = arena_records(E, g, arena);
        const double term = E.logtab[n1];
        int4 clo = make_int4(0, -1, 0, 0), chi = make_int4(0, 0, -1, 0);
        double best;
        const int4 nohi = make_int4(0, 0, -1, 0);
        const int bi = scan_children<false, W, true>(E, R, nullptr, lo, nohi, term, lane, clo, chi, r, &best);
        if (lane == 0) {
            pre->clo = clo;
            pre->chi = chi;
            pre->best = best;
            pre->term = term;
            pre->besti = bi;
        }
    }
    if (lane == 0) pre->valid = ok ? 1 : 0;
}

template <bool VL, int W = kWords, class Hook = NoHook>
__device__ __forceinline__ void select_body(const Dev &E, float *obs, int g, int lane, int j = 0, uint64_t *lds_leaf = nullptr,
                                            Hook *hook = nullptr) {
    static_assert(!(Hook::kOn && VL), "the root pre-scan is the sequential search's");
    const int gk = VL ? g * E.K + j : g;
    const int arena = E.cur_arena[g];
    const int top0 = E.top[g];
    int to_move = E.root_to_move[g];
    int last = E.root_last[g];
    const bool act = E.active[g] != 0;
    const int S = E.S;
    uint64_t st[2][kWords];
    load_board<W>(E.root_stones, g, st);
    uint64_t window = 0;
    window = E.line_tab[lane];
    uint64_t window_hi = 0;
    if constexpr (W == 2) window_hi = E.line_tab[kWave + lane];
    RootPre was = {};
    bool pre_ok = false;
    int4 st_lo = make_int4(0, -1, 0, 0);
    int st_r = 0, st_scan = 0;
    if constexpr (Hook::kOn) {
        was = *hook->pre;
        pre_ok = __builtin_amdgcn_readfirstlane(was.scan != 0 && was.valid != 0 ? 1 : 0) != 0;
    }
    if (!act) return;
    int4 *R = arena_records(E, g, arena);
    const float *P = arena_priors(E, g, arena);
    const bool use_puct = E.score_mode == RZ_SCORE_PUCT;
    int top = top0;
    int nst = count_bits<W>(st[0]) + count_bits<W>(st[1]);

    int32_t *path = E.path + (long long)gk * E.path_stride;
    int node = 0, depth = 0, fresh = 0;
    if (lane == 0) path[0] = 0;

    int4 lo = R[0], hi = R[1];
    int4 plo = lo, phi = hi;
    if constexpr (Hook::kOn) {
        const int s = pre_ok ? was.lo.y + was.r : 0;
        plo = R[2 * s];
        phi = R[2 * s + 1];
        hook->root_cell(last, nst, lane);
        hook->tick(0, lo.x);
    }
    for (int it = 0; it <= S; ++it) {
        const int k = rec_k(lo);
        if (k == 0) break;
        int fc = lo.y;
        int r;
        int4 clo = make_int4(0, -1, 0, 0), chi = make_int4(0, 0, -1, 0);
        if (use_puct) {
            r = scan_children<true, W>(E, R, P, lo, hi, sqrt((double)lo.x), lane, clo, chi);
        } else if (lo.z < k) {
            const int nv = lo.z;
            int cap = rec_cap(lo);
            if (nv == cap) {
                const int ncap = cap == 0 ? (k < kFirstCap ? k : kFirstCap) : (2 * cap < k ? 2 * cap : k);
                if ((long long)top + ncap > E.cap) {
                    flag(E, g, RZ_FLAG_ARENA_FULL, lane);
                    fresh = 2;
                    break;
                }
                for (int i = lane; i < nv; i += kWave) {
                    const int4 a = R[2 * (fc + i)], b = R[2 * (fc + i) + 1];
                    R[2 * (top + i)] = a;
                    R[2 * (top + i) + 1] = b;
                }
                if (VL) {
                    for (int jj = 0; jj < j; ++jj) {
                        const int gj = g * E.K + jj;
                        int32_t *pj = E.path + (long long)gj * E.path_stride;
                        const int dj = E.leaf_depth[gj];
                        for (int d = lane; d <= dj; d += kWave) {
                            const int q = pj[d];
                            if (q >= fc && q < fc + nv) pj[d] = q - fc + top;
                        }
                        if (lane == 0) {
                            const int q = E.leaf_node[gj];
                            if (q >= fc && q < fc + nv) E.leaf_node[gj] = q - fc + top;
                        }
                    }
                }
                fc = top;
                top += ncap;
                cap = ncap;
            }
            r = nv;
            fresh = 1;
            if constexpr (Hook::kOn) {
                if (it == 0) st_lo = make_int4(lo.x, fc, nv + 1, pack_kc(k, cap));
            }
            if (lane == 0) {
                R[2 * node] = make_int4(lo.x + (VL ? 1 : 0), fc, nv + 1, pack_kc(k, cap));
                if (VL) {
                    *rec_wsum(R, node) = rec_w(hi) - 1.0;
                    R[2 * (fc + r)] = make_int4(1, -1, 0, 0);
                    R[2 * (fc + r) + 1] = make_hi(-1.0, -1, 0.0f);
                }
            }
        } else {
            const int pn = lo.x;
            if (pn < 1 || pn >= E.logtab_n) {
                flag(E, g, RZ_FLAG_LOGTAB, lane);
                break;
            }
            bool answered = false;
            int r_pre = 0;
            if constexpr (Hook::kOn) {
                if (it == 0 && pre_ok && lo.x == was.lo.x + 1 && lo.y == was.lo.y && lo.z == was.lo.z && lo.w == was.lo.w) {
                    const double sr = uct_ref(rec_w(phi), plo.x, was.term, E.c_puct);
                    const bool cand = sr > -INFINITY, none = was.besti == 0x7fffffff;
                    const bool mine = cand && (none || sr > was.best || (sr == was.best && was.r < was.besti));
                    const bool take = __builtin_amdgcn_readfirstlane(mine ? 1 : 0) != 0;
                    r_pre = __builtin_amdgcn_readfirstlane(take ? was.r : was.besti);
                    const int4 wlo = take ? plo : was.clo, whi = take ? phi : was.chi;
                    clo = make_int4(__builtin_amdgcn_readfirstlane(wlo.x), __builtin_amdgcn_readfirstlane(wlo.y),
                                    __builtin_amdgcn_readfirstlane(wlo.z), __builtin_amdgcn_readfirstlane(wlo.w));
                    chi = make_int4(__builtin_amdgcn_readfirstlane(whi.x), __builtin_amdgcn_readfirstlane(whi.y),
                                    __builtin_amdgcn_readfirstlane(whi.z), __builtin_amdgcn_readfirstlane(whi.w));
                    if (lane == 0) hook->pre->answered += 1;
                    answered = true;
                }
            }
            r = answered ? r_pre : scan_children<false, W>(E, R, P, lo, hi, E.logtab[pn], lane, clo, chi);
            if constexpr (Hook::kOn) {
                if (it == 0) st_lo = lo;
            }
        }
        if constexpr (Hook::kOn) {
            if (it == 0) hook->tick(1, r);
        }
        if (r >= k) {
            flag(E, g, RZ_FLAG_INTERNAL, lane);
            break;
        }
        if (VL && !fresh && lane == 0) {
            *rec_n(R, node) = lo.x + 1;
            *rec_wsum(R, node) = rec_w(hi) - 1.0;
        }
        uint64_t occ[kWords];
#pragma unroll
        for (int j = 0; j < kWords; ++j) occ[j] = st[0][j] | st[1][j];
        const Legal L = legal_of<W>(E, occ, lane);
        int action, cell;
        if (!nth_legal<W>(E, occ, L, r, lane, action, cell)) {
            flag(E, g, RZ_FLAG_INTERNAL, lane);
            break;
        }
        if constexpr (Hook::kOn) {
            hook->cell(depth, cell, lane);
            if (it == 0) {
                st_r = r;
                st_scan = !use_puct && st_lo.z == k ? 1 : 0;
                hook->tick(2, cell);
            }
        }
        if (to_move == 0) set_bit<W>(st[0], cell); else set_bit<W>(st[1], cell);
        last = cell;
        to_move ^= 1;
        nst += 1;
        node = fc + r;
        depth += 1;
        if (lane == 0) path[depth] = node;
        if (fresh) break;
        lo = clo;
        hi = chi;
    }
    if constexpr (Hook::kOn) {
        hook->tick(3, node);
        hook->depth = depth;
        if (lane == 0) {
            RootPre *pre = hook->pre;
            pre->lo = st_lo;
            pre->r = st_r;
            pre->scan = st_scan;
            pre->arena = arena;
        }
    }
    if (lane == 0 && top != top0) E.top[g] = top;
    if (VL && fresh != 1 && lane == 0) {
        *rec_n(R, node) = lo.x + 1;
        *rec_wsum(R, node) = rec_w(hi) - 1.0;
    }

    int term = 0;
    double tval = 0.0;
    {
        int winner = -1;
        if (depth == 0) {
            if (line_anywhere<W>(st[0], S, E.BH, E.BW, E.n_row, lane, E.bw_rcp)) winner = 0;
            else if (line_anywhere<W>(st[1], S, E.BH, E.BW, E.n_row, lane, E.bw_rcp)) winner = 1;
        } else {
            const int mover = to_move ^ 1;
            if (line_through<W>(mover == 0 ? st[0] : st[1], last, E.BH, E.BW, E.n_row, lane, E.bw_rcp, E.n_rcp, window, window_hi, E.line_masks != 0)) winner = mover;
        }
        if (winner >= 0) {
            term = 2;
            tval = (winner == to_move) ? 1.0 : -1.0;
        } else if (nst == S) {
            term = 1;
            tval = 0.0;
        }
    }
    if (lane == 0) {
        E.leaf_node[gk] = node;
        E.leaf_depth[gk] = depth;
        E.leaf_fresh[gk] = fresh;
        E.leaf_term[gk] = term;
        E.leaf_tval[gk] = tval;
        E.leaf_to_move[gk] = to_move;
        E.leaf_last[gk] = last;
    }
    store_board<W>(E.leaf_stones, gk, st, lane);
    if (lds_leaf != nullptr) {
        store_board<W>(lds_leaf, 0, st, lane);
        if (lane == 0) {
            reinterpret_cast<int *>(lds_leaf + 2 * kWords)[0] = to_move;
            reinterpret_cast<int *>(lds_leaf + 2 * kWords)[1] = last;
        }
    }
    if constexpr (Hook::kOn) hook->tick(4, term);
    if (obs != nullptr)
        write_obs(obs + (long long)gk * 4 * S, to_move == 0 ? st[0] : st[1],
                  to_move == 0 ? st[1] : st[0], last, nst, S, lane);
}

typedef rz_raw_heads RawHeads;
typedef rz_value_head ValueHead;
constexpr int kDefWaves = 4;

template <typename VT, bool PROBS = false, bool RAW = false, bool VL = false, bool DEF = false, int W = kWords>
__device__ __forceinline__ void expand_backup_body(const Dev &E, const float *logp, const VT *value, int g,
                                                   int lane, RawHeads rh = RawHeads(), int j = 0, ValueHead vh = ValueHead(),
                                                   float (*part)[kWave] = nullptr) {
    const int gk = VL ? g * E.K + j : g;
    const int slot = DEF ? E.pend[g] : 0;
    const bool act = E.active[g] != 0;
    const int arena = E.cur_arena[g];
    const int depth = E.leaf_depth[gk];
    const int fresh = E.leaf_fresh[gk];
    const int term = E.leaf_term[gk];
    const double leaf_tval = E.leaf_tval[gk];
    const int ptop = E.ptop[g];
    const int nblk = E.nblk[g];
    const int top_now = E.top[g];
    const int noise_ctr = E.noise_ctr[g];
    const int leaf_tm = DEF ? E.leaf_to_move[gk] : 0, leaf_lc = DEF ? E.leaf_last[gk] : 0;
    const int32_t *path = E.path + (long long)gk * E.path_stride;
    const int path_lane = path[lane < E.path_stride ? lane : 0];
    uint64_t st[2][kWords];
    load_board<W>(E.leaf_stones, gk, st);
    float lse = 0.0f, raw_value = 0.0f;
    float x[kWords] = {0.f, 0.f, 0.f, 0.f};
    if (RAW) {
        const float *r = rh.raw + (size_t)gk * rh.ld;
        const float *hp = rh.hid + (size_t)gk * 64 + lane;
        const float w2 = rh.w2[lane], b2 = rh.b2[0];
        float hid = hp[0];
        float mx = -INFINITY;
        if (rh.n_parts == 4) {
            const long long rs = rh.raw_part_stride, hs = rh.hid_part_stride;
            const float act_scale = rh.act_scale[0], val_scale = rh.val_scale[0];
            float part[kWords][4], bias[kWords];
#pragma unroll
            for (int i = 0; i < kWords; ++i) {
                const int j = lane + 64 * i;
                const bool in = j < E.A;
#pragma unroll
                for (int q = 0; q < 4; ++q) part[i][q] = in ? r[j + q * rs] : 0.0f;
                bias[i] = in ? rh.act_bias[j] : 0.0f;
            }
            const float h1 = hp[hs], h2 = hp[2 * hs], h3 = hp[3 * hs], hb = rh.val_bias[lane];
#pragma unroll
            for (int i = 0; i < kWords; ++i) {
                const float sum4 = ((part[i][0] + part[i][1]) + part[i][2]) + part[i][3];
                x[i] = lane + 64 * i < E.A ? fmaf(sum4, act_scale, bias[i]) : -INFINITY;
                mx = fmaxf(mx, x[i]);
            }
            hid = fmaxf(fmaf(((hid + h1) + h2) + h3, val_scale, hb), 0.0f);
        } else {
#pragma unroll
            for (int i = 0; i < kWords; ++i) {
                const int j = lane + 64 * i;
                x[i] = j < E.A ? r[j] : -INFINITY;
                mx = fmaxf(mx, x[i]);
            }
        }
        mx = wave_max(mx, lane);
        float sum = 0.0f;
#pragma unroll
        for (int i = 0; i < kWords; ++i) sum += (lane + 64 * i < E.A) ? expf(x[i] - mx) : 0.0f;
        sum = wave_sum(sum, lane);
        lse = mx + logf(sum);
        float h = hid * w2;
        h = wave_sum(h, lane);
        raw_value = tanhf(h + b2);
    }
    float def_value = 0.0f;
    if (DEF) {
        const float b1 = vh.b1[lane], w2 = vh.w2[lane], b2 = vh.b2[0];
        __syncthreads();
        float hid = part[0][lane];
#pragma unroll
        for (int q = 1; q < kDefWaves; ++q) hid += part[q][lane];
        hid = fmaxf(hid + b1, 0.0f);
        def_value = tanhf(wave_sum(hid * w2, lane) + b2);
    }
    if (!act) return;
    int4 *R = arena_records(E, g, arena);
    float *P = arena_priors(E, g, arena);

    const double v = term ? leaf_tval : (DEF ? (double)def_value : RAW ? (double)raw_value : (double)value[gk]);
    if (DEF && slot >= E.pend_cap) {
        flag(E, g, RZ_FLAG_INTERNAL, lane);
        return;
    }
    const long long rec = DEF ? (long long)slot * E.n_games + g : 0;

    int new_fc = -1, new_nv = 0, new_k = 0, new_cap = 0, new_pb = -1;
    bool expand_now = !term && fresh != 2;
    if (VL && expand_now) {
        const int leaf = __shfl(path_lane, depth < kWave ? depth : 0);
        expand_now = rec_k(R[2 * (depth < kWave ? leaf : path[depth])]) == 0;
    }
    if (expand_now) {
        uint64_t occ[kWords];
#pragma unroll
        for (int j = 0; j < kWords; ++j) occ[j] = st[0][j] | st[1][j];
        const Legal L = legal_of<W>(E, occ, lane);
        const int k = L.k;
        const bool dense = !DEF && E.score_mode == RZ_SCORE_PUCT;
        const int top = dense ? top_now : 0;
        if ((long long)ptop + k > E.pcap || nblk >= E.qcap) {
            flag(E, g, RZ_FLAG_BLOCKS_FULL, lane);
        } else if (dense && (long long)top + k > E.cap) {
            flag(E, g, RZ_FLAG_ARENA_FULL, lane);
        } else {
            new_pb = ptop;
            new_k = k;
            if (dense) {
                new_fc = top;
                new_nv = k;
                new_cap = k;
            }
            if (lane == 0) {
                E.ptop[g] = ptop + k;
                E.nblk[g] = nblk + 1;
                if (dense) E.top[g] = top + k;
            }
            if (DEF) {
                if (lane == 0) {
                    E.pend_pb[rec] = ptop;
                    E.pend_ctr[rec] = noise_ctr;
                    E.pend_lw[rec] = pend_lw_pack(leaf_tm, leaf_lc);
                    if (E.add_noise) E.noise_ctr[g] = noise_ctr + 1;
                }
                store_board<W>(E.pend_stones, (int)rec, st, lane);
            }
            const float uniform = 1.0f / (float)k;
            if (!DEF) {
            int ranks[kWords];
            int before = 0;
#pragma unroll
            for (int j = 0; j < kWords; ++j) ranks[j] = lane_action_rank(E, occ, L, j, lane, before);
            float noise[kWords] = {0.f, 0.f, 0.f, 0.f};
            float noise_sum = 1.0f;
            if (E.add_noise) {
                const int ctr = noise_ctr;
                const uint64_t key = mix64(mix64(E.noise_key[g]) ^ (uint64_t)ctr);
                float local = 0.0f;
#pragma unroll
                for (int j = 0; j < kWords; ++j)
                    if (ranks[j] >= 0) {
                        noise[j] = gamma03(hash32((uint32_t)key ^ (uint32_t)(key >> 32)) + 0x9E3779B9u * (uint32_t)(64 * j + lane + 1));
                        local += noise[j];
                    }
                local = wave_sum(local, lane);
                noise_sum = local > 0.0f ? local : 1.0f;
                if (lane == 0) E.noise_ctr[g] = ctr + 1;
            }
#pragma unroll
            for (int j = 0; j < kWords; ++j) {
                const int r = ranks[j];
                if (r < 0) continue;
                const int a = 64 * j + lane;
                float prior = uniform;
                if (RAW) prior = expf(x[j] - lse);
                else if (logp) prior = PROBS ? logp[(long long)gk * E.A + a] : expf(logp[(long long)gk * E.A + a]);
                if (E.add_noise) prior = 0.75f * prior + 0.25f * (noise[j] / noise_sum);
                P[ptop + r] = prior;
                if (dense) {
                    R[2 * (top + r)] = make_int4(0, -1, 0, 0);
                    R[2 * (top + r) + 1] = make_hi(0.0, -1, prior);
                }
            }
            }
        }
    }
    if (DEF && lane == 0) {
        if (new_pb < 0) E.pend_pb[rec] = -1;
        E.pend[g] = slot + 1;
    }

    for (int d = lane; d <= depth; d += kWave) {
        const int node = d == lane ? path_lane : path[d];
        const double x = ((depth - d) & 1) ? v : -v;
        if (VL) {
            if (d == depth && new_k > 0) {
                const int4 m = R[2 * node];
                R[2 * node] = make_int4(m.x, new_fc, new_nv, pack_kc(new_k, new_cap));
                *rec_pb(R, node) = new_pb;
            }
            *rec_wsum(R, node) += x + 1.0;
        } else if (d == depth) {
            if (fresh == 1) {
                R[2 * node] = make_int4(1, new_fc, new_nv, pack_kc(new_k, new_cap));
                R[2 * node + 1] = make_hi(0.0 + x, new_pb, 0.0f);
            } else {
                const int4 m = R[2 * node];
                R[2 * node] = (new_k > 0) ? make_int4(m.x + 1, new_fc, new_nv, pack_kc(new_k, new_cap))
                                          : make_int4(m.x + 1, m.y, m.z, m.w);
                *rec_wsum(R, node) += x;
                if (new_k > 0) *rec_pb(R, node) = new_pb;
            }
        } else {
            *rec_n(R, node) += 1;
            *rec_wsum(R, node) += x;
        }
    }
}

template <int PER>
__device__ __forceinline__ void value_quarter_def(const ValueHead &vh, int gk, int lane, int q, float (*part)[kWave]) {
    typedef float vec4 __attribute__((ext_vector_type(4)));
    typedef const __attribute__((address_space(4))) vec4 *uniform_row;
    const vec4 *w = reinterpret_cast<const vec4 *>(vh.w1t) + (size_t)q * 2 * PER * kWave + lane;
    const uniform_row f = (uniform_row)(reinterpret_cast<const vec4 *>(vh.valfeat + (size_t)gk * vh.ld) + q * 2 * PER);
    float a0 = 0.0f, a1 = 0.0f;
#pragma unroll
    for (int half = 0; half < 2; ++half) {
        vec4 wv[PER], fv[PER];
#pragma unroll
        for (int i = 0; i < PER; ++i) {
            wv[i] = w[(size_t)(half * PER + i) * kWave];
            fv[i] = f[half * PER + i];
        }
#pragma unroll
        for (int i = 0; i < PER; ++i) {
            a0 = fmaf(fv[i].x, wv[i].x, a0);
            a1 = fmaf(fv[i].y, wv[i].y, a1);
            a0 = fmaf(fv[i].z, wv[i].z, a0);
            a1 = fmaf(fv[i].w, wv[i].w, a1);
        }
        __builtin_amdgcn_sched_barrier(0);
    }
    part[q][lane] = a0 + a1;
}

template <int PER>
__device__ __forceinline__ void value_quarter_lds(const ValueHead &vh, const float *row, int lane, int q, float (*part)[kWave]) {
    typedef float vec4 __attribute__((ext_vector_type(4)));
    const vec4 *w = reinterpret_cast<const vec4 *>(vh.w1t) + (size_t)q * 2 * PER * kWave + lane;
    const vec4 *f = reinterpret_cast<const vec4 *>(row) + q * 2 * PER;
    float a0 = 0.0f, a1 = 0.0f;
#pragma unroll
    for (int half = 0; half < 2; ++half) {
        vec4 wv[PER], fv[PER];
#pragma unroll
        for (int i = 0; i < PER; ++i) {
            wv[i] = w[(size_t)(half * PER + i) * kWave];
            fv[i] = f[half * PER + i];
        }
#pragma unroll
        for (int i = 0; i < PER; ++i) {
            a0 = fmaf(fv[i].x, wv[i].x, a0);
            a1 = fmaf(fv[i].y, wv[i].y, a1);
            a0 = fmaf(fv[i].z, wv[i].z, a0);
            a1 = fmaf(fv[i].w, wv[i].w, a1);
        }
        __builtin_amdgcn_sched_barrier(0);
    }
    part[q][lane] = a0 + a1;
}

}
}
```

Before: 24.93 million.

## Overlap wave-0 selection tail with early release; wave 0 runs conv1 alone

Wave 0 now releases the other waves partway through tree selection through a hook. It then builds the leaf's input planes and conv1 lists itself and runs all conv1 tiles alone. Waves 1-3 split the base-record gathers three ways, using precomputed per-word counts. This removes one block barrier and the serial hand-over, so selection's tail overlaps with the gather. In exchange wave 0 carries more serial conv1 work, the per-wave gather rounds grow, and correctness depends on the new release and leaf hooks.

```diff
diff --git a/profiles/microbench/delta_resident_phases.py b/profiles/microbench/delta_resident_phases.py
--- a/profiles/microbench/delta_resident_phases.py
+++ b/profiles/microbench/delta_resident_phases.py
@@ -8,10 +8,11 @@
 from rlzero_amd.engine import HipNetEvaluator, MCTSEngine
 from rlzero_amd.games.gomoku.policy_value_net import PolicyValueNet
 lib = H.load()
-NAMES = [(0, 'leaf + changed cells'), (1, 'distances, requests, ranks'), (3, 'maps, base records'), (4, 'bar'), (5, 'conv1'), (6, 'bar'), (7, 'conv2'),
+NAMES = [(0, 'verdict'), (1, 'requests, ranks'), (3, 'maps; wave 0: planes, conv1'), (4, 'bar'), (5, 'conv1'), (6, 'bar'), (7, 'conv2'),
          (9, 'bar + conv3 + heads'), (10, 'bar'), (11, 'features'), (12, 'bar'), (16, 'value layer'), (17, 'expand + backup'),
-         (2, 'sel: root record'), (8, 'sel: root scan / answer'), (13, 'sel: level-0 cell'), (14, 'sel: deeper levels'), (15, 'sel: terminal test + leaf stores'),
-         (18, 'selection (rest: hand-over)'), (19, 'wave 1: pre-scan'), (20, 'wave 1: wait behind it')]
+         (2, 'sel: root record'), (8, 'sel: root scan / answer'), (13, 'sel: level-0 cell'), (14, 'sel: deeper levels'), (15, 'sel: tail behind the release'),
+         (18, 'selection (up to the release)'), (19, 'wave 1: pre-scan'), (20, 'wave 1: wait behind it'),
+         (21, 'wave 1: release -> its arrival at the barrier before conv2')]
 VALUES = '--values' in sys.argv[1:]
 if VALUES:
     import rlzero_amd.route as _R
diff --git a/rlzero_amd/csrc/rz_delta.h b/rlzero_amd/csrc/rz_delta.h
--- a/rlzero_amd/csrc/rz_delta.h
+++ b/rlzero_amd/csrc/rz_delta.h
@@ -284,6 +284,7 @@
 
 struct Leaf {
     f16x4 cell_planes;
+    const uint64_t *leaf_lds;
     const char *base;
     int dys[kMaxD], dxs[kMaxD];
     _Float16 *dst16;
@@ -344,6 +345,56 @@
               "rz_gather.h's records are the base's and the budget is this file's");
 static_assert(rzg::kC1Bytes <= P1 && rzg::kC2Bytes <= P2, "a record fits its LDS slot");
 
+__device__ __forceinline__ f16x4 planes_of(const uint64_t (&ls)[8], int tid, int tm_eff, bool has_last, int lc, int par_count);
+
+__device__ __forceinline__ void leaf_from_lds(const uint64_t *leaf_lds, uint64_t (&ls)[8], int &tm, int &lc, int &nst) {
+    nst = 0;
+#pragma unroll
+    for (int q = 0; q < 8; ++q) {
+        ls[q] = uni64(leaf_lds[q]);
+        nst += __popcll(ls[q]);
+    }
+    tm = __builtin_amdgcn_readfirstlane(reinterpret_cast<const int *>(leaf_lds + 2 * RZ_BOARD_WORDS)[0]);
+    lc = __builtin_amdgcn_readfirstlane(reinterpret_cast<const int *>(leaf_lds + 2 * RZ_BOARD_WORDS)[1]);
+}
+
+__device__ __forceinline__ void conv1_tile(int tile, int total, int lane, const char *in0, const uint16_t *list1, const uint32_t *map1,
+                                           const sp::f16x8 (&a1)[3][2], const f32x4 (&bias1)[4], float k1, float act1) {
+    const int n32 = lane & 31, h = lane >> 5, idx = 32 * tile + n32;
+    const int pos = list1[idx];
+    const int py = (pos * 3641) >> 16, px = pos - py * kRowW;
+    typedef const __attribute__((address_space(3))) f16x4 *lds_half;
+    const lds_half q = (lds_half)(in0 + ((py - 1) * sp::kInCols + (px - 1) + 2 * h) * 8);
+    sp::f16x8 b1[3];
+#pragma unroll
+    for (int ky = 0; ky < 3; ++ky) {
+        const int o = ky * sp::kInCols;
+        const f16x4 lo4 = q[o], hi4 = q[o + 1];
+        b1[ky] = __builtin_shufflevector(lo4, hi4, 0, 1, 2, 3, 4, 5, 6, 7);
+    }
+    sp::f32x16 acc1;
+#pragma unroll
+    for (int r = 0; r < 16; ++r) acc1[r] = 0.0f;
+#pragma unroll
+    for (int ky = 0; ky < 3; ++ky)
+#pragma unroll
+        for (int combo = 0; combo < 3; combo += 2)
+            acc1 = __builtin_amdgcn_mfma_f32_32x32x16_f16(a1[ky][combo == 2], b1[ky], acc1, 0, 0, 0);
+    if (idx < total) {
+        const uint32_t rec = map1[pos] + (uint32_t)(4 * h * 2);
+#pragma unroll
+        for (int gg = 0; gg < 4; ++gg) {
+            float z[4];
+#pragma unroll
+            for (int j = 0; j < 4; ++j) z[j] = fmaxf(fmaf(acc1[4 * gg + j], k1, bias1[gg][j] * act1), 0.0f);
+            f16x4 hi, lo;
+            sp::split4(z, hi, lo);
+            *(lds_h4)(uintptr_t)(rec + 8 * gg * 2) = hi;
+            *(lds_h4)(uintptr_t)(rec + 8 * gg * 2 + 64) = lo;
+        }
+    }
+}
+
 template <bool SETS, int OLO = 0, int OHI = 6>
 __device__ __forceinline__ int delta_passes(const NetDev &nd, const DeltaArgs &da, char *lds, int tid0, int wave, const Leaf &leaf, const Layers &ly,
                                             f32x4 headv, bool &use_delta, Prof &prof) {
@@ -355,7 +406,6 @@
     const float k1 = ly.k1, k2 = ly.k2, k3 = ly.k3, act1 = ly.act1, act2 = ly.act2, act3 = ly.act3;
     const char *t2p = ly.t2p, *t3p = ly.t3p;
     const char *base = leaf.base;
-    const f16x4 cell_planes = leaf.cell_planes;
     const int (&dys)[kMaxD] = leaf.dys, (&dxs)[kMaxD] = leaf.dxs;
     _Float16 *dst16 = leaf.dst16;
     float *vdst = leaf.vdst, *dst32 = leaf.dst32;
@@ -405,45 +455,9 @@
         const bool g1 = pass < 0 && f[3] && !f[0], g2 = pass < 0 && f[4] && !f[1];
         const __amdgpu_buffer_rsrc_t b_rsrc = __builtin_amdgcn_make_buffer_rsrc(const_cast<char *>(base), 0, kBaseBytes, 0x00020000);
         f32x4 r1[8], r2[16];
-        f32x4 q1[rzg::kC1Rounds], q2[rzg::kC2Rounds];
-        uint32_t d1[rzg::kC1Rounds], d2[rzg::kC2Rounds];
-        if constexpr (SETS) {
-            uint16_t *tab = leaf.gtab;
-            uint64_t ws[rzw::kRadii][rzg::kWords];
-#pragma unroll
-            for (int r = 0; r < rzw::kRadii; ++r)
-#pragma unroll
-                for (int w = 0; w < rzg::kWords; ++w) ws[r][w] = leaf.sets[4 * r + w];
-            int n1 = 0, s1 = 0, n2 = 0, s2 = 0;
-#pragma unroll
-            for (int w = 0; w < rzg::kWords; ++w) {
-                const uint64_t h1 = rzg::held(ws[2][w], ws[0][w]), h2 = rzg::held(ws[3][w], ws[1][w]);
-                const int cell = 64 * w + lane;
-                const int p1 = rzg::c1_place(n1 + lane_below(h1), wave), p2 = rzg::c2_place(n2 + lane_below(h2), wave);
-                const uint16_t e1 = rzg::entry(cell, s1 + lane_below(ws[2][w])), e2 = rzg::entry(cell, s2 + lane_below(ws[3][w]));
-                if (handed && ((h1 >> lane) & 1ull) && p1 >= 0) tab[p1] = e1;
-                if (handed && ((h2 >> lane) & 1ull) && p2 >= 0) tab[p2] = e2;
-                n1 += rzg::popcount(h1), s1 += rzg::popcount(ws[2][w]);
-                n2 += rzg::popcount(h2), s2 += rzg::popcount(ws[3][w]);
-            }
-            const uint32_t c1a = lds_addr(c1), c2a = lds_addr(c2);
-#pragma unroll
-            for (int i = 0; i < rzg::kC1Rounds; ++i) {
-                const int j = rzg::c1_record(i, wave, lane), chunk = rzg::c1_chunk(lane);
-                const uint16_t e = tab[rzg::c1_index(j)];
-                const bool has = handed && rzg::c1_has(j, n1);
-                d1[i] = has ? c1a + (uint32_t)rzg::dst(rzg::entry_slot(e), chunk, P1) : zaddr + 16u * (uint32_t)chunk;
-                q1[i] = load_rec(b_rsrc, rzg::c1_src(has, rzg::entry_cell(e), chunk));
-            }
-#pragma unroll
-            for (int i = 0; i < rzg::kC2Rounds; ++i) {
-                const int j = rzg::c2_record(i, wave, lane), chunk = rzg::c2_chunk(lane);
-                const uint16_t e = tab[rzg::c2_index(j)];
-                const bool has = handed && rzg::c2_has(j, n2);
-                d2[i] = has ? c2a + (uint32_t)rzg::dst(rzg::entry_slot(e), chunk, P2) : zaddr + 16u * (uint32_t)chunk;
-                q2[i] = load_rec(b_rsrc, rzg::c2_src(has, rzg::entry_cell(e), chunk, (int)kBaseC2));
-            }
-        } else {
+        typedef rzg::Split<SETS ? 3 : 4> GS;
+        constexpr int NW = SETS ? 3 : 4;
+        if constexpr (!SETS) {
             const int o1 = g1 ? tid * 128 : kOutside, o2 = g2 ? (int)kBaseC2 + tid * 256 : kOutside;
 #pragma unroll
             for (int i = 0; i < 8; ++i) r1[i] = load_rec(b_rsrc, o1 + 16 * i);
@@ -461,7 +475,7 @@
         if constexpr (SETS) {
             const __amdgpu_buffer_rsrc_t s_rsrc = __builtin_amdgcn_make_buffer_rsrc(const_cast<f32x4 *>(nd.s1), 0, 6 * 64 * 16, 0x00020000);
             const __amdgpu_buffer_rsrc_t o_rsrc = __builtin_amdgcn_make_buffer_rsrc(const_cast<float *>(nd.b1), 0, 32 * 4, 0x00020000);
-            const bool runs = !handed || 32 * wave < tot[0];
+            const bool runs = !handed || wave == 0;
             const int so = runs ? lane * 16 : kOutside, bo = runs ? 16 * (lane >> 5) : kOutside;
 #pragma unroll
             for (int ky = 0; ky < 3; ++ky)
@@ -517,13 +531,74 @@
         if (f[0]) list1[rank[0]] = (uint16_t)mypos;
         if (f[1]) list2[rank[1]] = (uint16_t)mypos;
         if (f[2]) list3[rank[2]] = (uint16_t)mypos;
-        if (pass <= 0 && is_cell) *reinterpret_cast<f16x4 *>(in0 + ((cy + 1) * sp::kInCols + (cx + 1)) * 8) = cell_planes;
+        if constexpr (SETS) {
+            if (!handed && pass <= 0) {
+                uint64_t ls[8];
+                int tm, lc, nst;
+                leaf_from_lds(leaf.leaf_lds, ls, tm, lc, nst);
+                const f16x4 planes = planes_of(ls, tid, tm, nst > 0, lc, nst);
+                if (is_cell) *reinterpret_cast<f16x4 *>(in0 + ((cy + 1) * sp::kInCols + (cx + 1)) * 8) = planes;
+            }
+        } else {
+            if (pass <= 0 && is_cell) *reinterpret_cast<f16x4 *>(in0 + ((cy + 1) * sp::kInCols + (cx + 1)) * 8) = leaf.cell_planes;
+        }
         if (pass <= 0 && store_head && tid < 226) reinterpret_cast<f32x4 *>(headw)[tid] = headv;
         if constexpr (SETS) {
-#pragma unroll
-            for (int i = 0; i < rzg::kC1Rounds; ++i) *(lds_v4)(uintptr_t)d1[i] = q1[i];
-#pragma unroll
-            for (int i = 0; i < rzg::kC2Rounds; ++i) *(lds_v4)(uintptr_t)d2[i] = q2[i];
+          if (!(handed && wave == 0)) {
+            f32x4 q1[GS::kC1Rounds], q2[GS::kC2Rounds];
+            uint32_t d1[GS::kC1Rounds], d2[GS::kC2Rounds];
+            uint16_t *tab = leaf.gtab;
+            const int gw = wave - 1, gwi = gw < 0 ? 0 : gw;
+            const bool gathers = handed && gw >= 0;
+            const int *wcnt = reinterpret_cast<const int *>(leaf.sets + kWinSets);
+            int pn1[rzg::kWords + 1], ps1[rzg::kWords + 1], pn2[rzg::kWords + 1], ps2[rzg::kWords + 1];
+            pn1[0] = ps1[0] = pn2[0] = ps2[0] = 0;
+#pragma unroll
+            for (int w = 0; w < rzg::kWords; ++w) {
+                const int k0 = __builtin_amdgcn_readfirstlane(wcnt[4 * 0 + w]), k1_ = __builtin_amdgcn_readfirstlane(wcnt[4 * 1 + w]);
+                const int k2_ = __builtin_amdgcn_readfirstlane(wcnt[4 * 2 + w]), k3_ = __builtin_amdgcn_readfirstlane(wcnt[4 * 3 + w]);
+                pn1[w + 1] = pn1[w] + k2_ - k0, ps1[w + 1] = ps1[w] + k2_;
+                pn2[w + 1] = pn2[w] + k3_ - k1_, ps2[w + 1] = ps2[w] + k3_;
+            }
+            const int n1 = pn1[rzg::kWords], n2 = pn2[rzg::kWords];
+            if (gathers) {
+                uint64_t ws[rzw::kRadii][rzg::kWords];
+#pragma unroll
+                for (int r = 0; r < rzw::kRadii; ++r)
+#pragma unroll
+                    for (int w = 0; w < rzg::kWords; ++w) ws[r][w] = leaf.sets[4 * r + w];
+#pragma unroll
+                for (int w = 0; w < rzg::kWords; ++w) {
+                    const uint64_t h1 = rzg::held(ws[2][w], ws[0][w]), h2 = rzg::held(ws[3][w], ws[1][w]);
+                    const int cell = 64 * w + lane;
+                    const int p1 = rzg::c1_place<NW>(pn1[w] + lane_below(h1), gw), p2 = rzg::c2_place<NW>(pn2[w] + lane_below(h2), gw);
+                    const uint16_t e1 = rzg::entry(cell, ps1[w] + lane_below(ws[2][w])), e2 = rzg::entry(cell, ps2[w] + lane_below(ws[3][w]));
+                    if (((h1 >> lane) & 1ull) && p1 >= 0) tab[p1] = e1;
+                    if (((h2 >> lane) & 1ull) && p2 >= 0) tab[p2] = e2;
+                }
+            }
+            const uint32_t c1a = lds_addr(c1), c2a = lds_addr(c2);
+#pragma unroll
+            for (int i = 0; i < GS::kC1Rounds; ++i) {
+                const int j = rzg::c1_record<NW>(i, gwi, lane), chunk = rzg::c1_chunk(lane);
+                const uint16_t e = tab[rzg::c1_index<NW>(j)];
+                const bool has = gathers && rzg::c1_has(j, n1);
+                d1[i] = has ? c1a + (uint32_t)rzg::dst(rzg::entry_slot(e), chunk, P1) : zaddr + 16u * (uint32_t)chunk;
+                q1[i] = load_rec(b_rsrc, rzg::c1_src(has, rzg::entry_cell(e), chunk));
+            }
+#pragma unroll
+            for (int i = 0; i < GS::kC2Rounds; ++i) {
+                const int j = rzg::c2_record<NW>(i, gwi, lane), chunk = rzg::c2_chunk(lane);
+                const uint16_t e = tab[rzg::c2_index<NW>(j)];
+                const bool has = gathers && rzg::c2_has(j, n2);
+                d2[i] = has ? c2a + (uint32_t)rzg::dst(rzg::entry_slot(e), chunk, P2) : zaddr + 16u * (uint32_t)chunk;
+                q2[i] = load_rec(b_rsrc, rzg::c2_src(has, rzg::entry_cell(e), chunk, (int)kBaseC2));
+            }
+#pragma unroll
+            for (int i = 0; i < GS::kC1Rounds; ++i) *(lds_v4)(uintptr_t)d1[i] = q1[i];
+#pragma unroll
+            for (int i = 0; i < GS::kC2Rounds; ++i) *(lds_v4)(uintptr_t)d2[i] = q2[i];
+          }
         } else {
             if (g1) {
 #pragma unroll
@@ -543,48 +618,42 @@
 #pragma unroll
                 for (int p = 0; p < 2; ++p) a2[tap][0][p] = sp::load_w(w_rsrc, lane * 16, (tap * 2 + p) * 1024);
         }
-        NET_TICK(3);
-        __syncthreads();
-        NET_TICK(4);
-
-        if (32 * wave < tot[0]) {
-            const int n32 = lane & 31, h = lane >> 5, idx = 32 * wave + n32;
-            const int pos = list1[idx];
-            const int py = (pos * 3641) >> 16, px = pos - py * kRowW;
-            typedef const __attribute__((address_space(3))) f16x4 *lds_half;
-            const lds_half q = (lds_half)(in0 + ((py - 1) * sp::kInCols + (px - 1) + 2 * h) * 8);
-            sp::f16x8 b1[3];
-#pragma unroll
-            for (int ky = 0; ky < 3; ++ky) {
-                const int o = ky * sp::kInCols;
-                const f16x4 lo4 = q[o], hi4 = q[o + 1];
-                b1[ky] = __builtin_shufflevector(lo4, hi4, 0, 1, 2, 3, 4, 5, 6, 7);
-            }
-            sp::f32x16 acc1;
-#pragma unroll
-            for (int r = 0; r < 16; ++r) acc1[r] = 0.0f;
-#pragma unroll
-            for (int ky = 0; ky < 3; ++ky)
-#pragma unroll
-                for (int combo = 0; combo < 3; combo += 2)
-                    acc1 = __builtin_amdgcn_mfma_f32_32x32x16_f16(a1[ky][combo == 2], b1[ky], acc1, 0, 0, 0);
-            if (idx < tot[0]) {
-                const uint32_t rec = map1[pos] + (uint32_t)(4 * h * 2);
-#pragma unroll
-                for (int gg = 0; gg < 4; ++gg) {
-                    float z[4];
-#pragma unroll
-                    for (int j = 0; j < 4; ++j) z[j] = fmaxf(fmaf(acc1[4 * gg + j], k1, bias1[gg][j] * act1), 0.0f);
-                    f16x4 hi, lo;
-                    sp::split4(z, hi, lo);
-                    *(lds_h4)(uintptr_t)(rec + 8 * gg * 2) = hi;
-                    *(lds_h4)(uintptr_t)(rec + 8 * gg * 2 + 64) = lo;
+        if (handed) {
+            if (wave == 0) {
+                uint64_t ls[8];
+                int tm, lc, nst;
+                leaf_from_lds(leaf.leaf_lds, ls, tm, lc, nst);
+                const int *cnt = reinterpret_cast<const int *>(leaf.sets + kWinSets);
+                int b0 = 0, b3 = 0;
+#pragma unroll
+                for (int w = 0; w < 4; ++w) {
+                    const int cell = 64 * w + lane, y = (cell * da.bw_rcp) >> 16, x = cell - y * BW;
+                    const f16x4 planes = planes_of(ls, cell, tm, nst > 0, lc, nst);
+                    if (cell < S) *reinterpret_cast<f16x4 *>(in0 + ((y + 1) * sp::kInCols + (x + 1)) * 8) = planes;
+                    const uint64_t w1 = uni64(leaf.sets[4 * 0 + w]), w3 = uni64(leaf.sets[4 * 2 + w]);
+                    const int pos = (y + 1) * kRowW + x + 1;
+                    if ((w1 >> lane) & 1ull) {
+                        list1[b0 + lane_below(w1)] = (uint16_t)pos;
+                        map1[pos] = lds_addr(c1 + (b3 + lane_below(w3)) * P1);
+                    }
+                    b0 += __builtin_amdgcn_readfirstlane(cnt[4 * 0 + w]);
+                    b3 += __builtin_amdgcn_readfirstlane(cnt[4 * 2 + w]);
                 }
-            }
-        }
-        NET_TICK(5);
-        __syncthreads();
-        NET_TICK(6);
+#pragma unroll 1
+                for (int tile = 0; 32 * tile < tot[0]; ++tile) conv1_tile(tile, tot[0], lane, in0, list1, map1, a1, bias1, k1, act1);
+            }
+            NET_TICK(3);
+            __syncthreads();
+            NET_TICK(4);
+        } else {
+            NET_TICK(3);
+            __syncthreads();
+            NET_TICK(4);
+            if (32 * wave < tot[0]) conv1_tile(wave, tot[0], lane, in0, list1, map1, a1, bias1, k1, act1);
+            NET_TICK(5);
+            __syncthreads();
+            NET_TICK(6);
+        }
         if (mode == 1 && f[0]) {
             f32x4 *dstp = reinterpret_cast<f32x4 *>(const_cast<char *>(base) + (size_t)tid * 128);
 #pragma unroll
@@ -798,7 +867,7 @@
     if (mode != 1 && !deferred && feat16 != nullptr)
         leaf.dst16 = feat16 + ((size_t)(board >> 5) * (nd.groups_act + nd.groups_val) * 1024 + (board & 31) * 16);
     leaf.dst32 = (mode != 1 && da.feat32 != nullptr) ? da.feat32 + (size_t)board * 6 * S : nullptr;
-    leaf.sets = nullptr, leaf.gtab = nullptr;
+    leaf.sets = nullptr, leaf.gtab = nullptr, leaf.leaf_lds = nullptr;
     leaf.deferred = deferred;
     leaf.store_head = true;
 
@@ -900,6 +969,29 @@
     __device__ __forceinline__ void cell(int level, int c, int lane) {
         const uint64_t v = win[c * kWinSets + (lane & (kWinSets - 1))];
         row = (lane >> 4) == level ? v : row;
+    }
+    uint64_t *leaf_lds, *ws;
+    bool base_ok, release;
+    __device__ __forceinline__ void leaf(const uint64_t (&st)[2][rzt::kWords], int to_move, int last, int d, int lane) {
+        depth = d;
+        rzt::store_board<rzt::kWords>(leaf_lds, 0, st, lane);
+        if (lane == 0) {
+            reinterpret_cast<int *>(leaf_lds + 2 * rzt::kWords)[0] = to_move;
+            reinterpret_cast<int *>(leaf_lds + 2 * rzt::kWords)[1] = last;
+        }
+        const bool mine = d == 0 ? (lane < 16 && any0) : (lane >> 4) < d;
+        const int nD = d == 0 ? (any0 ? 1 : 0) : d;
+        windows_store(mine ? row : 0ull, base_ok && nD <= kMaxD, d & 1, nD, lane, ws);
+        if (release) __syncthreads();
+#ifdef RZ_NET_PROFILE
+        {
+            __builtin_amdgcn_sched_barrier(0);
+            const long long now = __builtin_readcyclecounter();
+            prof->acc[18] += now - prof->t;
+            prof->t = now;
+            __builtin_amdgcn_sched_barrier(0);
+        }
+#endif
     }
 #ifdef RZ_NET_PROFILE
     Prof *prof;
@@ -919,20 +1011,14 @@
 #endif
 };
 
-__device__ __forceinline__ void path_windows(const ResHook &hook, bool base_ok, int lane, uint64_t *ws) {
-    const int depth = hook.depth;
-    const bool mine = depth == 0 ? (lane < 16 && hook.any0) : (lane >> 4) < depth;
-    const int nD = depth == 0 ? (hook.any0 ? 1 : 0) : depth;
-    windows_store(mine ? hook.row : 0ull, base_ok && nD <= kMaxD, depth & 1, nD, lane, ws);
-}
-
 constexpr int kResVrow = 512;
 template <bool POL>
 __global__ __launch_bounds__(256, 2) void k_delta_res(NetDev nd, _Float16 *__restrict__ store16, DeferredOut later, DeltaArgs da, ResArgs<true> res) {
     __shared__ __attribute__((aligned(16))) char lds[kLdsBytes];
     __shared__ float res_vrow[kResVrow];
     __shared__ float res_part[rzt::kDefWaves][rzt::kWave];
-    static_assert(rzg::kTabEntries * 2 <= rzt::kWave * 4, "a wave's gather table lies in its row of the K-quarter sums");
+    static_assert(rzg::Split<3>::kTabEntries == 14 * 4 + 6 * 8 && rzg::Split<3>::kTabEntries <= 128 && rzg::Split<3>::kTabEntries * 2 <= rzt::kWave * 4,
+                  "a gathering wave's table (104 entries) lies in its 128-entry row of the K-quarter sums");
     __shared__ __attribute__((aligned(16))) uint64_t res_leaf[2 * RZ_BOARD_WORDS + 2];
     __shared__ __attribute__((aligned(16))) uint64_t res_win[kWinLds / 8];
     __shared__ __attribute__((aligned(16))) rzt::RootPre res_pre;
@@ -985,6 +1071,10 @@
     hook.depth = 0;
     hook.any0 = false;
     hook.row = 0ull;
+    hook.leaf_lds = res_leaf;
+    hook.ws = res_win;
+    hook.base_ok = base_ok;
+    hook.release = false;
 #ifdef RZ_NET_PROFILE
     hook.prof = &prof;
     long long pre_cycles = 0, pre_wait = 0;
@@ -1000,7 +1090,6 @@
         const int lane0 = tid0 & 63;
         if (res.select_first != 0) {
             rzt::select_body<false, rzt::kWords, ResHook>(res.E, nullptr, game, lane0, 0, res_leaf, &hook);
-            path_windows(hook, base_ok, lane0, res_win);
         } else {
             leaf_windows(res_leaf, rs, base_ok, h_tm, da, BW, lane0, res_win);
         }
@@ -1010,17 +1099,6 @@
     for (int sim = 0; sim < n_sims; ++sim) {
         int tid_s = tid0;
         asm volatile("" : "+v"(tid_s));
-        uint64_t ls[8];
-        int nst = 0;
-#pragma unroll
-        for (int q = 0; q < 8; ++q) {
-            const uint64_t v = res_leaf[q];
-            ls[q] = ((uint64_t)(unsigned)__builtin_amdgcn_readfirstlane((int)(v >> 32)) << 32) | (unsigned)__builtin_amdgcn_readfirstlane((int)v);
-            nst += __popcll(ls[q]);
-        }
-        const int tm = __builtin_amdgcn_readfirstlane(reinterpret_cast<const int *>(res_leaf + 2 * RZ_BOARD_WORDS)[0]);
-        const int lc = __builtin_amdgcn_readfirstlane(reinterpret_cast<const int *>(res_leaf + 2 * RZ_BOARD_WORDS)[1]);
-        const bool has_last = nst > 0;
         const int verdict = __builtin_amdgcn_readfirstlane(reinterpret_cast<const int *>(res_win + kWinSets)[kWinSets]);
         bool use_delta = (verdict & 1) != 0;
         const int parity = (verdict >> 1) & 1, nD = verdict >> 8;
@@ -1030,7 +1108,7 @@
 #pragma unroll
         for (int i = 0; i < kMaxD; ++i) leaf.dys[i] = leaf.dxs[i] = -100;
         leaf.base = da.recs + ((size_t)game * 2 + parity) * kBaseBytes;
-        leaf.cell_planes = planes_of(ls, tid_s, tm, has_last, lc, nst);
+        leaf.leaf_lds = res_leaf;
         leaf.dst16 = POL && slot0 + sim < later.n_slots ? store16 + (size_t)(slot0 + sim) * later.slot_halfs + (size_t)(game >> 5) * nd.groups_act * 1024 + (game & 31) * 16 : nullptr;
         leaf.vdst = res_vrow;
         leaf.dst32 = nullptr;
@@ -1072,16 +1150,20 @@
         if (RZ_DELTA_PRESCAN && wave == 1 && more) pre_wait += __builtin_readcyclecounter();
 #endif
         NET_TICK(17);
-        if (wave == 0 && more) {
-            hook.depth = 0, hook.any0 = false, hook.row = 0ull;
-            int lane_t = lane;
-            asm volatile("" : "+v"(lane_t));
-            rzt::select_body<false, rzt::kWords, ResHook>(res.E, nullptr, game, lane_t, 0, res_leaf, &hook);
-            path_windows(hook, base_ok, lane_t, res_win);
+        if (more) {
+            if (wave == 0) {
+                hook.depth = 0, hook.any0 = false, hook.row = 0ull;
+                hook.release = true;
+                int lane_t = lane;
+                asm volatile("" : "+v"(lane_t));
+                rzt::select_body<false, rzt::kWords, ResHook>(res.E, nullptr, game, lane_t, 0, res_leaf, &hook);
+                NET_TICK(15);
+            } else {
+                __syncthreads();
+                NET_TICK(18);
+            }
         }
         if (RZ_DELTA_TREE_PRIO) __builtin_amdgcn_s_setprio(0);
-        __syncthreads();
-        NET_TICK(18);
     }
     if (da.stats != nullptr && tid0 == 0) {
         atomicAdd(da.stats + 0, (unsigned)deltas);
@@ -1098,13 +1180,14 @@
 #ifdef RZ_NET_PROFILE
     if (blockIdx.x == 0 && tid0 == 0) {
         for (int i = 0; i < 24; ++i)
-            if (i != 19 && i != 20) net_prof[i] = prof_acc[i];
+            if (i != 19 && i != 20 && i != 21) net_prof[i] = prof_acc[i];
         net_prof[23] = __builtin_readcyclecounter() - prof_k0;
         net_prof[22] = tiles_total;
     }
     if (blockIdx.x == 0 && tid0 == 64) {
         net_prof[19] = pre_cycles;
         net_prof[20] = pre_wait;
+        net_prof[21] = prof_acc[0] + prof_acc[1] + prof_acc[3];
     }
 #endif
 }
@@ -1174,7 +1257,7 @@
         leaf.dst16 = store16 + (size_t)slot * pr.slot_halfs + (size_t)(game >> 5) * nd.groups_act * 1024 + (game & 31) * 16;
         leaf.vdst = nullptr;
         leaf.dst32 = nullptr;
-        leaf.sets = nullptr, leaf.gtab = nullptr;
+        leaf.sets = nullptr, leaf.gtab = nullptr, leaf.leaf_lds = nullptr;
         leaf.deferred = false;
         leaf.store_head = first;
         first = false;
diff --git a/rlzero_amd/csrc/rz_gather.h b/rlzero_amd/csrc/rz_gather.h
--- a/rlzero_amd/csrc/rz_gather.h
+++ b/rlzero_amd/csrc/rz_gather.h
@@ -14,11 +14,21 @@
 constexpr int kC1Bytes = 128, kC2Bytes = 256;
 constexpr int kC1Lanes = kC1Bytes / 16, kC2Lanes = kC2Bytes / 16;
 constexpr int kC1PerWave = 64 / kC1Lanes, kC2PerWave = 64 / kC2Lanes;
-constexpr int kC1PerRound = 4 * kC1PerWave, kC2PerRound = 4 * kC2PerWave;
-constexpr int kC1Rounds = (kC1Max + kC1PerRound - 1) / kC1PerRound;
-constexpr int kC2Rounds = (kC2Max + kC2PerRound - 1) / kC2PerRound;
-constexpr int kTabC2 = 0, kTabC1 = kC2Rounds * kC2PerWave;
-constexpr int kTabEntries = kTabC1 + kC1Rounds * kC1PerWave;
+template <int NW>
+struct Split {
+    static constexpr int kC1PerRound = NW * kC1PerWave, kC2PerRound = NW * kC2PerWave;
+    static constexpr int kC1Rounds = (kC1Max + kC1PerRound - 1) / kC1PerRound;
+    static constexpr int kC2Rounds = (kC2Max + kC2PerRound - 1) / kC2PerRound;
+    static constexpr int kTabC2 = 0, kTabC1 = kC2Rounds * kC2PerWave;
+    static constexpr int kTabEntries = kTabC1 + kC1Rounds * kC1PerWave;
+};
+constexpr int kC1PerRound = Split<4>::kC1PerRound, kC2PerRound = Split<4>::kC2PerRound;
+constexpr int kC1Rounds = Split<4>::kC1Rounds;
+constexpr int kC2Rounds = Split<4>::kC2Rounds;
+constexpr int kTabC2 = Split<4>::kTabC2, kTabC1 = Split<4>::kTabC1;
+constexpr int kTabEntries = Split<4>::kTabEntries;
+static_assert(kC1Rounds == 4 && kC2Rounds == 11 && kTabEntries == 76, "the four-wave split");
+static_assert(Split<3>::kC1Rounds == 6 && Split<3>::kC2Rounds == 14 && Split<3>::kTabEntries == 104, "the three-wave split: 164 / 12 and 128 / 24 rounds");
 constexpr int kOutside = 1 << 30;
 
 RZG_FN int popcount(uint64_t w) { return __builtin_popcountll(w); }
@@ -45,22 +55,22 @@
     return -1;
 }
 
-RZG_FN int c2_record(int round, int wave, int lane) { return kC2PerRound * round + kC2PerWave * wave + (int)((unsigned)lane / kC2Lanes); }
+template <int NW = 4> RZG_FN int c2_record(int round, int wave, int lane) { return Split<NW>::kC2PerRound * round + kC2PerWave * wave + (int)((unsigned)lane / kC2Lanes); }
 RZG_FN int c2_chunk(int lane) { return (int)((unsigned)lane % kC2Lanes); }
-RZG_FN int c1_record(int round, int wave, int lane) { return kC1PerRound * round + kC1PerWave * wave + (int)((unsigned)lane / kC1Lanes); }
+template <int NW = 4> RZG_FN int c1_record(int round, int wave, int lane) { return Split<NW>::kC1PerRound * round + kC1PerWave * wave + (int)((unsigned)lane / kC1Lanes); }
 RZG_FN int c1_chunk(int lane) { return (int)((unsigned)lane % kC1Lanes); }
-RZG_FN int c2_rounds(int n) { return (n + kC2PerRound - 1) / kC2PerRound; }
-RZG_FN int c1_rounds(int n) { return (n + kC1PerRound - 1) / kC1PerRound; }
+template <int NW = 4> RZG_FN int c2_rounds(int n) { return (n + Split<NW>::kC2PerRound - 1) / Split<NW>::kC2PerRound; }
+template <int NW = 4> RZG_FN int c1_rounds(int n) { return (n + Split<NW>::kC1PerRound - 1) / Split<NW>::kC1PerRound; }
 
-RZG_FN int c2_wave(int j) { return (int)(((unsigned)j / kC2PerWave) % 4u); }
-RZG_FN int c2_index(int j) { return kTabC2 + (int)(((unsigned)j / kC2PerRound) * kC2PerWave + (unsigned)j % kC2PerWave); }
-RZG_FN int c1_wave(int j) { return (int)(((unsigned)j / kC1PerWave) % 4u); }
-RZG_FN int c1_index(int j) { return kTabC1 + (int)(((unsigned)j / kC1PerRound) * kC1PerWave + (unsigned)j % kC1PerWave); }
+template <int NW = 4> RZG_FN int c2_wave(int j) { return (int)(((unsigned)j / kC2PerWave) % (unsigned)NW); }
+template <int NW = 4> RZG_FN int c2_index(int j) { return Split<NW>::kTabC2 + (int)(((unsigned)j / Split<NW>::kC2PerRound) * kC2PerWave + (unsigned)j % kC2PerWave); }
+template <int NW = 4> RZG_FN int c1_wave(int j) { return (int)(((unsigned)j / kC1PerWave) % (unsigned)NW); }
+template <int NW = 4> RZG_FN int c1_index(int j) { return Split<NW>::kTabC1 + (int)(((unsigned)j / Split<NW>::kC1PerRound) * kC1PerWave + (unsigned)j % kC1PerWave); }
 RZG_FN uint16_t entry(int cell, int slot) { return (uint16_t)(cell | slot << 8); }
 RZG_FN int entry_cell(uint16_t e) { return e & 255; }
 RZG_FN int entry_slot(uint16_t e) { return e >> 8; }
-RZG_FN int c2_place(int j, int wave) { return j < kC2Max && c2_wave(j) == wave ? c2_index(j) : -1; }
-RZG_FN int c1_place(int j, int wave) { return j < kC1Max && c1_wave(j) == wave ? c1_index(j) : -1; }
+template <int NW = 4> RZG_FN int c2_place(int j, int wave) { return j < kC2Max && c2_wave<NW>(j) == wave ? c2_index<NW>(j) : -1; }
+template <int NW = 4> RZG_FN int c1_place(int j, int wave) { return j < kC1Max && c1_wave<NW>(j) == wave ? c1_index<NW>(j) : -1; }
 
 RZG_FN int c2_src(bool has, int cell, int chunk, int base_c2) { return has ? base_c2 + cell * kC2Bytes + 16 * chunk : kOutside; }
 RZG_FN int c1_src(bool has, int cell, int chunk) { return has ? cell * kC1Bytes + 16 * chunk : kOutside; }
diff --git a/rlzero_amd/csrc/rz_tree.h b/rlzero_amd/csrc/rz_tree.h
--- a/rlzero_amd/csrc/rz_tree.h
+++ b/rlzero_amd/csrc/rz_tree.h
@@ -689,9 +689,9 @@
         lo = clo;
         hi = chi;
     }
+    if constexpr (Hook::kOn) hook->leaf(st, to_move, last, depth, lane);
     if constexpr (Hook::kOn) {
         hook->tick(3, node);
-        hook->depth = depth;
         if (lane == 0) {
             RootPre *pre = hook->pre;
             pre->lo = st_lo;
@@ -735,7 +735,7 @@
         E.leaf_last[gk] = last;
     }
     store_board<W>(E.leaf_stones, gk, st, lane);
-    if (lds_leaf != nullptr) {
+    if (!Hook::kOn && lds_leaf != nullptr) {
         store_board<W>(lds_leaf, 0, st, lane);
         if (lane == 0) {
             reinterpret_cast<int *>(lds_leaf + 2 * kWords)[0] = to_move;
```

Result: faster. 25.71 million (median of 6 runs) (+3.1%).
